# peterropac/Aegolius

Hardware: AMD Instinct MI355X
Metric: Mpoints/sec SDF eval, 1024^3 grid, 10-prim smooth-union tree (higher is better)
Workload: dtype f32

## Files before the change

### aegolius_amd/_engine.py

```python
import atexit
import contextlib
import ctypes
import importlib.util
import os
import sys
import threading

import numpy as np

_HERE = os.path.dirname(os.path.abspath(__file__))
LIB_PATH = os.path.join(_HERE, "libsdfk.so")

MODE_AUTO, MODE_INTERPRET, MODE_SPECIALIZED, MODE_NOCULL = 0, 1, 2, 3
(FLAVOUR_PLAIN_ARRAY, FLAVOUR_PLAIN_GRID, FLAVOUR_TILE_ARRAY, FLAVOUR_TILE_GRID, FLAVOUR_TILE_MASK, FLAVOUR_ROWS_ARRAY,
 FLAVOUR_ROWS_GRID, FLAVOUR_ROWS_MASK, FLAVOUR_ROWS2D_ARRAY, FLAVOUR_ROWS2D_GRID, FLAVOUR_RAYS, FLAVOUR_OCCUPANCY) = range(12)
FLAVOUR_FLAGS = 0x100
FLAVOUR_XY = 0x200

_c = ctypes
_vp, _i64, _int, _sz = _c.c_void_p, _c.c_int64, _c.c_int, _c.c_size_t
_fp = _c.POINTER(_c.c_float)

SIGNATURES = {
    "sdfk_abi_version": (_int, []),
    "sdfk_device_count": (_int, []),
    "sdfk_last_error": (_c.c_char_p, []),
    "sdfk_program_create": (_vp, [_vp, _sz, _vp, _sz, _vp, _sz, _int]),
    "sdfk_program_destroy": (None, [_vp]),
    "sdfk_program_set_params": (_int, [_vp, _vp, _sz]),
    "sdfk_program_set_cull": (_int, [_vp, _vp, _sz, _vp]),
    "sdfk_program_source": (_c.c_char_p, [_vp]),
    "sdfk_program_compile_check": (_int, [_vp, _c.POINTER(_sz)]),
    "sdfk_program_chain_members": (_int, [_vp]),
    "sdfk_program_compile_flavour": (_int, [_vp, _int, _c.POINTER(_sz), _c.POINTER(_c.c_double)]),
    "sdfk_debug_compile_external": (_int, [_vp, _int, _c.POINTER(_sz)]),
    "sdfk_debug_jit_stats": (None, [_c.POINTER(_i64), _c.POINTER(_c.c_double)]),
    "sdfk_jit_drain": (None, []),
    "sdfk_jit_cancel": (None, []),
    "sdfk_debug_set_rtc_defs": (None, [_c.c_char_p]),
    "sdfk_eval_device": (_int, [_vp, _vp, _i64, _i64, _vp, _vp, _int]),
    "sdfk_eval_device_rows": (_int, [_vp, _vp, _i64, _i64, _i64, _vp, _vp, _int]),
    "sdfk_eval_device_rows2d": (_int, [_vp, _vp, _i64, _i64, _i64, _vp, _vp, _int]),
    "sdfk_eval_device_rows2d_xy": (_int, [_vp, _vp, _i64, _i64, _i64, _vp, _vp, _int]),
    "sdfk_debug_cells_stats": (None, [_int, _c.POINTER(_c.c_longlong)]),
    "sdfk_debug_rays_stats": (None, [_int, _c.POINTER(_c.c_longlong)]),
    "sdfk_eval_device_rows3d": (_int, [_vp, _vp, _i64, _i64, _i64, _i64, _i64, _vp, _vp, _int]),
    "sdfk_debug_row_masks": (_int, [_vp, _vp, _i64, _i64, _i64, _vp, _c.POINTER(_i64), _c.POINTER(_int), _vp]),
    "sdfk_eval_grid_sharded": (_int, [_vp, _vp, _i64, _vp, _i64, _vp, _i64, _int, _vp, _vp, _int]),
    "sdfk_eval_grid_sharded_device": (_int, [_vp, _vp, _i64, _vp, _i64, _vp, _i64, _int, _vp, _int, _vp, _int]),
    "sdfk_eval_device_aux": (_int, [_vp, _vp, _i64, _i64, _vp, _int, _i64, _vp, _vp, _int]),
    "sdfk_eval_grid_aux": (_int, [_vp, _vp, _i64, _vp, _i64, _vp, _i64, _i64, _i64, _vp, _int, _i64, _vp, _vp, _int]),
    "sdfk_field_min": (_int, [_vp, _i64, _c.POINTER(_c.c_float), _vp]),
    "sdfk_grid_box_average": (_int, [_vp, _i64, _i64, _i64, _int, _int, _int, _int, _vp, _vp]),
    "sdfk_grid_edge_detect": (_int, [_vp, _i64, _i64, _i64, _vp, _vp]),
    "sdfk_debug_box_variant": (_int, [_i64, _i64, _i64, _int, _int, _int, _c.POINTER(_int)]),
    "sdfk_grid_signed": (_int, [_vp, _i64, _i64, _i64, _c.c_float, _int, _vp, _vp]),
    "sdfk_grid_boundary_mask": (_int, [_vp, _i64, _c.c_float, _vp, _vp]),
    "sdfk_grid_signed_slab": (_int, [_vp, _i64, _i64, _vp, _i64, _i64, _i64, _int, _vp, _vp]),
    "sdfk_eval_host": (_int, [_vp, _vp, _int, _i64, _i64, _vp, _int, _int]),
    "sdfk_eval_host_resident": (_int, [_vp, _vp, _int, _i64, _i64, _vp, _int, _int]),
    "sdfk_field_select_scratch": (_sz, [_i64]),
    "sdfk_field_select": (_int, [_vp, _i64, _c.c_float, _vp, _i64, _c.POINTER(_i64), _vp, _vp]),
    "sdfk_field_select_finish": (_int, [_i64, _i64, _vp, _i64, _vp, _vp]),
    "sdfk_field_gradient": (_int, [_vp, _i64, _i64, _i64, _int, _int, _vp, _i64, _vp]),
    "sdfk_field_crossings_2d": (_int, [_vp, _vp, _i64, _i64, _i64, _c.c_double, _c.c_double, _c.c_double, _vp, _vp]),
    "sdfk_lcwg_eval": (_int, [_int, _vp, _vp, _i64, _i64, _i64, _c.c_double, _c.c_double, _int, _c.c_double, _vp, _vp, _i64,
                              _vp]),
    "sdfk_lcwg_old_eval": (_int, [_int, _vp, _i64, _vp, _i64, _c.c_double, _c.c_double, _vp, _i64, _vp]),
    "sdfk_eval_select_scratch": (_sz, [_i64, _i64]),
    "sdfk_eval_device_select": (_int, [_vp, _vp, _i64, _i64, _i64, _int, _c.c_float, _vp, _i64, _c.POINTER(_i64), _vp, _vp, _int]),
    "sdfk_eval_grid_select": (_int, [_vp, _vp, _i64, _vp, _i64, _vp, _i64, _i64, _i64, _c.c_float, _vp, _i64, _c.POINTER(_i64),
                                     _vp, _vp, _int]),
    "sdfk_eval_select_finish": (_int, [_vp, _i64, _i64, _int, _i64, _vp, _i64, _vp, _vp]),
    "sdfk_vec_eval_device": (_int, [_vp, _int, _vp, _i64, _i64, _vp, _int, _i64, _int, _vp, _i64, _vp]),
    "sdfk_vec_set_interpret": (None, [_int]),
    "sdfk_vec_source": (_c.c_char_p, [_vp, _int, _int, _int]),
    "sdfk_vec_compile_check": (_int, [_vp, _int, _int, _int, _c.POINTER(_sz)]),
    "sdfk_vec_eval_host": (_int, [_vp, _int, _vp, _int, _i64, _vp, _i64, _vp, _i64, _vp, _i64, _vp, _int, _int, _vp, _int]),
    "sdfk_eval_grid": (_int, [_vp, _vp, _i64, _vp, _i64, _vp, _i64, _i64, _i64, _vp, _vp, _int]),
    "sdfk_eval_grid_host": (_int, [_vp, _vp, _i64, _vp, _i64, _vp, _i64, _i64, _i64, _vp, _int, _int]),
    "sdfk_set_default_mode": (None, [_int]),
    "sdfk_debug_brick_masks": (_int, [_vp, _vp, _i64, _i64, _vp, _vp]),
    "sdfk_linspace_f32": (_int, [_c.c_double, _c.c_double, _i64, _vp]),
    "sdfk_point_tree_build": (_i64, [_vp, _i64, _int, _vp, _i64, _vp, _vp, _vp]),
    "sdfk_grid_fill": (_int, [_vp, _i64, _vp, _i64, _vp, _i64, _vp, _i64, _i64, _i64, _vp]),
    "sdfk_set_device": (_int, [_int]),
    "sdfk_malloc": (_vp, [_sz]),
    "sdfk_free": (_int, [_vp]),
    "sdfk_memcpy_h2d": (_int, [_vp, _vp, _sz]),
    "sdfk_memcpy_d2h": (_int, [_vp, _vp, _sz]),
    "sdfk_memcpy_d2d": (_int, [_vp, _vp, _sz]),
    "sdfk_sync": (_int, [_vp]),
    "sdfk_event_create": (_vp, []),
    "sdfk_event_destroy": (_int, [_vp]),
    "sdfk_event_record": (_int, [_vp, _vp]),
    "sdfk_event_elapsed_ms": (_int, [_vp, _vp, _fp]),
    "sdfk_stream_probe": (_int, [_vp, _i64, _i64, _vp, _vp]),
    "sdfk_dual_has_rule": (_int, [_int]),
    "sdfk_program_jvp_check": (_int, [_vp, _c.POINTER(_int)]),
    "sdfk_eval_jvp_device": (_int, [_vp, _vp, _i64, _i64, _vp, _int, _int, _vp, _vp, _i64, _vp]),
    "sdfk_value_jvp_device": (_int, [_int, _vp, _vp, _vp, _i64, _vp, _vp, _vp]),
    "sdfk_program_vjp_check": (_int, [_vp, _c.POINTER(_int), _c.POINTER(_i64)]),
    "sdfk_vjp_limits": (_int, [_c.POINTER(_int), _c.POINTER(_int)]),
    "sdfk_eval_vjp_device": (_int, [_vp, _vp, _i64, _i64, _vp, _int, _int, _vp, _vp, _vp, _vp]),
    "sdfk_points_bin": (_int, [_vp, _i64, _i64, _vp, _i64, _i64, _i64, _vp, _vp]),
    "sdfk_points_extent": (_int, [_vp, _i64, _i64, _i64, _vp, _vp]),
    "sdfk_points_fill": (_int, [_vp, _i64, _i64, _i64, _int, _i64, _i64, _i64, _vp]),
    "sdfk_points_widen": (_int, [_vp, _i64, _int, _vp, _vp]),
    "sdfk_field_isosurface_scratch": (_sz, [_i64, _i64, _i64]),
    "sdfk_field_isosurface": (_int, [_vp, _vp, _i64, _vp, _i64, _vp, _i64, _c.c_float, _c.POINTER(_i64), _c.POINTER(_i64), _vp,
                                     _vp]),
    "sdfk_field_isosurface_finish": (_int, [_vp, _i64, _i64, _i64, _c.c_float, _i64, _i64, _vp, _i64, _vp, _i64, _int, _vp,
                                            _vp]),
    "sdfk_field_contour2d_scratch": (_sz, [_i64, _i64]),
    "sdfk_field_contour2d": (_int, [_vp, _vp, _i64, _vp, _i64, _c.c_float, _c.POINTER(_i64), _c.POINTER(_i64), _vp, _vp]),
    "sdfk_field_contour2d_finish": (_int, [_vp, _i64, _i64, _c.c_float, _i64, _i64, _vp, _i64, _vp, _i64, _int, _vp, _vp]),
    "sdfk_eval_grid_isosurface_scratch": (_sz, [_i64, _i64, _i64]),
    "sdfk_eval_grid_isosurface": (_int, [_vp, _vp, _i64, _vp, _i64, _vp, _i64, _c.c_float, _c.POINTER(_i64), _c.POINTER(_i64),
                                         _vp, _vp, _int]),
    "sdfk_eval_grid_isosurface_finish": (_int, [_vp, _vp, _i64, _vp, _i64, _vp, _i64, _c.c_float, _i64, _i64, _vp, _i64, _vp,
                                                _i64, _int, _vp, _vp, _int]),
    "sdfk_eval_grid_contour2d_scratch": (_sz, [_i64, _i64]),
# ... 660 lines not shown
```

### aegolius_amd/csrc/sdfk.hip

```cpp
#include <hip/hip_runtime.h>
#include <hip/hiprtc.h>

#include <chrono>
#include <algorithm>
#include <atomic>
#include <cmath>
#include <condition_variable>
#include <cstdio>
#include <cstdlib>
#include <cstring>
#include <deque>
#include <functional>
#include <map>
#include <memory>
#include <mutex>
#include <thread>
#include <string>
#include <vector>
#include <dirent.h>
#include <dlfcn.h>
#include <fcntl.h>
#include <signal.h>
#include <spawn.h>
#include <sys/wait.h>
// ... 985 lines not shown
        std::unique_lock<std::mutex> lk(mu);
        cv.wait(lk, [this] { return jobs.empty() && busy == 0; });
    }
    void drop_queued() {
        std::lock_guard<std::mutex> lk(mu);
        jobs.clear();
        cv.notify_all();
    }
    ~BuildWorker() {
        {
            std::lock_guard<std::mutex> lk(mu);
            stop = true;
            cv.notify_all();
        }
        for (std::thread& t : threads)
            if (t.joinable()) t.join();
    }
};
static BuildWorker g_builds;
extern "C" void sdfk_jit_drain(void) { g_builds.drain(); }
extern "C" void sdfk_jit_cancel(void) {
    g_cancel_builds.store(true);
    g_builds.drop_queued();
    g_builds.drain();
}
static std::atomic<long long> g_compile_count{0};
static std::atomic<long long> g_compile_micros{0};
extern "C" void sdfk_debug_jit_stats(int64_t* builds, double* seconds) {
    if (builds) *builds = g_compile_count.load();
    if (seconds) *seconds = (double)g_compile_micros.load() * 1e-6;
}

static std::shared_ptr<CodeObject> code_entry(const std::string& key) {
    std::lock_guard<std::mutex> lk(g_code_mu);
    std::shared_ptr<CodeObject>& e = g_code[key];
    if (!e) e = std::make_shared<CodeObject>();
    return e;
}
static void code_build(const std::shared_ptr<CodeObject>& e, const std::string& src, int rwb, bool external = false) {
    const auto t0 = std::chrono::steady_clock::now();
    std::vector<char> co;
    std::string log;
    bool from_disk = false;
    std::string disk_path;
    const int rc = rtc_compile(src, &co, &log, rwb, &from_disk, &disk_path, external);
    const double dt = std::chrono::duration<double>(std::chrono::steady_clock::now() - t0).count();
    if (!from_disk) {
        g_compile_count++;
        g_compile_micros += (long long)(dt * 1e6);
    }
    std::lock_guard<std::mutex> lk(e->mu);
    e->build_seconds = dt;
    if (rc == 0) {
        e->co.swap(co);
        e->disk_path = disk_path;
        e->state = 2;
    } else {
        e->error = log;
        e->state = 3;
        e->failed_at = std::chrono::steady_clock::now();
    }
    e->cv.notify_all();
}
template <typename MakeSource>
static std::shared_ptr<CodeObject> code_get(const std::string& key, MakeSource make_source, int rwb, bool wait) {
    std::shared_ptr<CodeObject> e = code_entry(key);
    std::unique_lock<std::mutex> lk(e->mu);
    if (e->state == 3 && std::chrono::steady_clock::now() - e->failed_at > std::chrono::seconds(30)) e->state = 0;
    if (e->state == 0) {
        e->state = 1;
        lk.unlock();
        const std::string src = make_source();
        if (wait || !rtc_helper_available()) {
            code_build(e, src, rwb);
        } else {
            g_builds.post([e, src, rwb] { code_build(e, src, rwb, true); });
        }
        return e;
    }
    if (wait) e->cv.wait(lk, [&] { return e->state != 1; });
    return e;
}
static std::string flavour_key(const sdfk_program* p, int flavour, int rwb, int with_flags = 0) {
    return p->key + "|f" + std::to_string(flavour) + ((with_flags & 1) ? "s" : "") + ((with_flags & 2) ? "x" : "") + "|" + rtc_option_key(rwb);
}
static std::string flavour_source(const sdfk_program* p, int flavour, int with_flags = 0) {
    return std::string((with_flags & 1) ? "#define SDFK_FLAGS 1\n" : "") + ((with_flags & 2) ? "#define SDFK_XY 1\n" : "") +
           sdfk_generate_source(g_ops, SDFK_OP_COUNT, p->code.data(), p->code.size() / 2, p->result_reg, p->sites, flavour,
                                &p->sites_all);
}

extern "C" int sdfk_program_chain_members(const sdfk_program* p) {
    return p && p->chain_mode ? p->chain_members : 0;
}
extern "C" int sdfk_program_compile_check(sdfk_program* p, size_t* code_size) {
    if (!p) return fail(-1, "null program");
    size_t total = 0;
    const int rwb = rows_geo(p);
    for (int f = 0; f < SDFK_FL_COUNT; ++f) {
        if (f == SDFK_FL_RAYS) continue;
        if (f == SDFK_FL_OCCUPANCY) continue;
        if (p->sites.empty() && f != SDFK_FL_PLAIN_ARRAY && f != SDFK_FL_PLAIN_GRID) continue;
        if (p->chain_mode && (f == SDFK_FL_TILE_ARRAY || f == SDFK_FL_TILE_GRID || f == SDFK_FL_TILE_MASK || f == SDFK_FL_ROWS_MASK)) continue;
        std::shared_ptr<CodeObject> e = code_get(flavour_key(p, f, rwb), [&] { return flavour_source(p, f); }, rwb, true);
        if (e->state != 2) return fail(-3, e->error);
        total += e->co.size();
    }
    if (code_size) *code_size = total;
    return 0;
}
extern "C" int sdfk_program_compile_flavour(sdfk_program* p, int flavour, size_t* code_size, double* seconds) {
    if (!p) return fail(-1, "null program");
    int with_flags = 0;
    if (flavour >= 0 && (flavour & SDFK_FLAVOUR_FLAGS)) with_flags |= 1;
    if (flavour >= 0 && (flavour & SDFK_FLAVOUR_XY)) with_flags |= 2;
    if (flavour >= 0) flavour &= ~(SDFK_FLAVOUR_FLAGS | SDFK_FLAVOUR_XY);
    if (flavour < 0 || flavour >= SDFK_FL_COUNT) return fail(-1, "sdfk_program_compile_flavour: unknown flavour");
    if (p->sites.empty() && flavour != SDFK_FL_PLAIN_ARRAY && flavour != SDFK_FL_PLAIN_GRID && flavour != SDFK_FL_RAYS &&
        flavour != SDFK_FL_OCCUPANCY)
        return fail(-2, "sdfk_program_compile_flavour: the program has no cull sites");
    if (with_flags && flavour == SDFK_FL_RAYS)
        return fail(-2, "sdfk_program_compile_flavour: the ray flavour has no flag-writing or two-row build");
    if (with_flags && flavour == SDFK_FL_OCCUPANCY)
        return fail(-2, "sdfk_program_compile_flavour: the occupancy flavour has no flag-writing or two-row build");
    if ((with_flags & 2) && flavour != SDFK_FL_PLAIN_ARRAY && flavour != SDFK_FL_ROWS2D_ARRAY)
        return fail(-2, "sdfk_program_compile_flavour: two-row coordinates exist for the plain and the flat row-block array kernels");
    if ((with_flags & 1) && (flavour == SDFK_FL_TILE_ARRAY || flavour == SDFK_FL_TILE_GRID || flavour == SDFK_FL_TILE_MASK ||
                       flavour == SDFK_FL_ROWS_MASK))
        return fail(-2, "sdfk_program_compile_flavour: this flavour has no flag-writing build");
    const int rwb = rows_geo(p);
    const auto t0 = std::chrono::steady_clock::now();
    std::shared_ptr<CodeObject> e =
        code_get(flavour_key(p, flavour, rwb, with_flags), [&] { return flavour_source(p, flavour, with_flags); }, rwb, true);
    if (e->state != 2) return fail(-3, e->error);
    if (code_size) *code_size = e->co.size();
    if (seconds) *seconds = std::chrono::duration<double>(std::chrono::steady_clock::now() - t0).count();
    return 0;
}

extern "C" int sdfk_debug_compile_external(sdfk_program* p, int flavour, size_t* code_size) {
    if (!p) return fail(-1, "null program");
    if (flavour < 0 || flavour >= SDFK_FL_COUNT) return fail(-1, "sdfk_debug_compile_external: unknown flavour");
    if (p->sites.empty() && flavour != SDFK_FL_PLAIN_ARRAY && flavour != SDFK_FL_PLAIN_GRID && flavour != SDFK_FL_RAYS &&
        flavour != SDFK_FL_OCCUPANCY)
        return fail(-2, "sdfk_debug_compile_external: the program has no cull sites");
    if (!rtc_helper_available()) return fail(-9, "sdfk_rtc_helper is not next to libsdfk.so (or hiprtc cannot be located)");
    std::vector<char> co;
    std::string log;
    if (rtc_compile_external(flavour_source(p, flavour), &co, &log, rows_geo(p)) != 0) return fail(-3, log);
    if (code_size) *code_size = co.size();
    return 0;
}

static std::shared_ptr<SpecModule> get_module(sdfk_program* p, int device, int flavour, bool wait, std::string* err,
                                              int with_flags = 0) {
    const int rwb = rows_geo(p);
    const std::string key = flavour_key(p, flavour, rwb, with_flags);
    std::shared_ptr<SpecModule> m;
    {
        std::lock_guard<std::mutex> lk(g_code_mu);
        std::shared_ptr<SpecModule>& slot = g_mods[std::make_pair(device, key)];
        if (!slot) slot = std::make_shared<SpecModule>();
        m = slot;
    }
    std::lock_guard<std::mutex> lk(m->mu);
    if (m->loaded) return m;
    for (int attempt = 0;; ++attempt) {
        std::shared_ptr<CodeObject> e;
        {
            std::lock_guard<std::mutex> ce(g_code_mu);
// ... 177 lines not shown
                 o_head = (o_cspan + 8 * nc + 63) & ~(size_t)63, o_pool = o_head + 2 * 64 * shards, total = o_pool + 4 * cap + 64;
    CellScratch* cs;
    {
        std::lock_guard<std::mutex> lk(p->mu);
        cs = &d->cells[stream];
    }
    if (cs->bytes < total) {
        if (cs->buf) {
            HIPCHK(hipStreamSynchronize(stream));
            (void)hipFree(cs->buf);
            cs->buf = nullptr;
            cs->bytes = 0;
        }
        if (hipMalloc(&cs->buf, total + total / 4) != hipSuccess) { (void)hipGetLastError(); return 0; }
        cs->bytes = total + total / 4;
    }
    char* b = cs->buf;
    HIPCHK(hipMemsetAsync(b + o_head, 0, 2 * 64 * shards, stream));
    CellPassArg cp{};
    cp.cand = b + o_pool;
    if (coarse) {
        cp.lv = crs; cp.parent = CellLevelH{}; cp.sph = b + o_csph; cp.span = b + o_cspan; cp.psph = nullptr; cp.pspan = nullptr;
        cp.ncells = (unsigned)nc; cp.inflate = 1.3f;
        cp.head = reinterpret_cast<unsigned*>(b + o_head);
        cp.base = 0u; cp.shard_cap = (unsigned)cshard;
        std::vector<void*> args = {(void*)&prm, (void*)&tab};
        for (int i = 0; i < n_src; ++i) args.push_back(src[i]);
        RowGeom g2 = rg;
        args.push_back(&g2);
        args.push_back(&cp);
        HIPCHK(hipModuleLaunchKernel(cells_fn, (unsigned)((nc + 3) / 4), 1, 1, 256, 1, 1, 0, stream, args.data(), nullptr));
    }
    cp.lv = fine; cp.parent = coarse ? crs : CellLevelH{}; cp.sph = b + o_fsph; cp.span = b + o_fspan;
    cp.psph = coarse ? b + o_csph : nullptr; cp.pspan = coarse ? b + o_cspan : nullptr;
    cp.ncells = (unsigned)nf; cp.inflate = 1.0f;
    cp.head = reinterpret_cast<unsigned*>(b + o_head + 64 * shards);
    cp.base = (unsigned)(shards * cshard); cp.shard_cap = (unsigned)fshard;
    {
        std::vector<void*> args = {(void*)&prm, (void*)&tab};
        for (int i = 0; i < n_src; ++i) args.push_back(src[i]);
        RowGeom g2 = rg;
        args.push_back(&g2);
        args.push_back(&cp);
        HIPCHK(hipModuleLaunchKernel(cells_fn, (unsigned)((nf + 3) / 4), 1, 1, 256, 1, 1, 0, stream, args.data(), nullptr));
    }
    static const bool trace = [] { const char* e = getenv("SDFK_CELLS_TRACE"); return e && e[0] == '1'; }();
    if (trace || g_cells_stats_on.load()) {
        HIPCHK(hipStreamSynchronize(stream));
        std::vector<uint2> sp(nf);
        unsigned head = 0;
        HIPCHK(hipMemcpy(sp.data(), b + o_fspan, 8 * nf, hipMemcpyDeviceToHost));
        {
            std::vector<unsigned> heads(2 * 16 * shards);
            HIPCHK(hipMemcpy(heads.data(), b + o_head, 2 * 64 * shards, hipMemcpyDeviceToHost));
            for (size_t i = 0; i < heads.size(); i += 16) head += heads[i];
        }
        unsigned long long sum = 0, all = 0, empty = 0, mx = 0;
        for (const uint2& x : sp) {
            if (x.y == 0xffffffffu) ++all;
            else { sum += x.y; mx = std::max<unsigned long long>(mx, x.y); if (x.y == 0) ++empty; }
        }
        {
            std::lock_guard<std::mutex> lk(g_cells_stats_mu);
            g_cells_stats[0] = (long long)nf; g_cells_stats[1] = (long long)nc; g_cells_stats[2] = (long long)head;
            g_cells_stats[3] = (long long)cap; g_cells_stats[4] = (long long)sum; g_cells_stats[5] = (long long)mx;
            g_cells_stats[6] = (long long)all; g_cells_stats[7] = (long long)empty;
        }
        if (trace) fprintf(stderr, "[sdfk cells] %d members: fine %ux%ux%u = %llu cells (2^%u planes x 2^%u blocks x 2^%u windows), coarse %llu; pool %u of %llu entries; "
                "fine lists: mean %.1f max %llu, %llu without a list, %llu empty\n", p->chain_members, fine.ncx, fine.ncy, fine.ncz, nf, fine.lx, fine.ly, fine.lz, nc,
                head, cap, (double)sum / (double)std::max<unsigned long long>(1, nf - all - empty), mx, all, empty);
    }
    out->lv = fine;
    out->sph = b + o_fsph;
    out->span = b + o_fspan;
    out->cand = b + o_pool;
    out->enabled = 1u;
    out->ncells = (unsigned)nf;
    return 0;
}

static int run(sdfk_program* p, const SrcArray* arr, const SrcGrid* grid, long long n, float* d_out, void* stream_,
               int mode, bool vec_ok, long long row_len = 0, const float* aux = nullptr, long long aux_stride = 0,
               bool flat = false, long long plane_rows = 0, long long plane_phase = 0, unsigned* d_flags = nullptr,
               unsigned thr_key = 0, bool xy = false) {
    if (!p) return fail(-1, "null program");
    if (n < 0) return fail(-1, "negative point count");
    if (p->n_aux > 0 && (!aux || aux_stride < n))
        return fail(-1, "this program reads auxiliary fields (staged evaluation): use sdfk_eval_device_aux / sdfk_eval_grid_aux");
    if (n == 0) return 0;
    if (mode == SDFK_MODE_AUTO) mode = g_default_mode;
    if (d_flags && (mode == SDFK_MODE_AUTO || mode == SDFK_MODE_INTERPRET)) mode = SDFK_MODE_SPECIALIZED;
    if (xy) {
        if (!arr || p->n_aux > 0) return fail(-1, "two-row coordinates: array source, no auxiliary fields");
        if (mode == SDFK_MODE_AUTO || mode == SDFK_MODE_INTERPRET) mode = SDFK_MODE_SPECIALIZED;
    }
    hipStream_t stream = (hipStream_t)stream_;
    int device = 0;
    HIPCHK(hipGetDevice(&device));
    DevState* d = nullptr;
    int rc = ensure_resident(p, device, stream, &d);
    if (rc) return rc;

    long long n4 = vec_ok ? (n / 4) * 4 : 0;
    long long tail = n - n4;

    static const long long spec_limit = [] {
        const char* e = getenv("SDFK_SPECIALIZE_LIMIT");
        const long long v = e ? atoll(e) : 1200;
        return v > 0 ? v : 1200;
    }();
    static const long long rows_limit = [] {
        const char* e = getenv("SDFK_ROWS_LIMIT");
        const long long v = e ? atoll(e) : 1200;
        return v > 0 ? v : 1200;
    }();
    if (mode == SDFK_MODE_AUTO && (long long)(p->code.size() / 2) > spec_limit && p->interp_ok && !p->chain_mode && !d_flags)
        mode = SDFK_MODE_INTERPRET;

    RowGeom rg;
    int flavour = arr ? SDFK_FL_PLAIN_ARRAY : SDFK_FL_PLAIN_GRID;
    const long long grow = grid ? (grid->n2 > 1 ? (long long)grid->n2 : (long long)grid->n1) : 0;
    if (!p->sites.empty() && mode != SDFK_MODE_NOCULL && mode != SDFK_MODE_INTERPRET) {
        if (arr && rows_geometry(n, row_len, &rg, (flat || d_flags) ? 0 : plane_rows, plane_phase, p->chain_mode))
            flavour = (flat || xy) ? SDFK_FL_ROWS2D_ARRAY : SDFK_FL_ROWS_ARRAY;
        else if (arr && vec_ok && !p->chain_mode && !d_flags && !xy) flavour = SDFK_FL_TILE_ARRAY;
        else if (grid && grid->start % grow == 0 &&
                 rows_geometry(n, grow, &rg, (grid->n2 > 1 && !d_flags) ? (long long)grid->n1 : 0,
                               grid->n2 > 1 ? (grid->start / grow) % (long long)grid->n1 : 0, p->chain_mode))
            flavour = grid->n2 > 1 ? SDFK_FL_ROWS_GRID : SDFK_FL_ROWS2D_GRID;
        else if (grid && vec_ok && !p->chain_mode && !d_flags) flavour = SDFK_FL_TILE_GRID;
        if (!p->chain_mode && (long long)(p->code.size() / 2) > rows_limit &&
            (flavour == SDFK_FL_ROWS_ARRAY || flavour == SDFK_FL_ROWS2D_ARRAY || flavour == SDFK_FL_ROWS_GRID || flavour == SDFK_FL_ROWS2D_GRID)) {
            const bool is_arr = arr != nullptr;
            if (vec_ok && !d_flags && !xy) flavour = is_arr ? SDFK_FL_TILE_ARRAY : SDFK_FL_TILE_GRID;
            else if (!d_flags) flavour = is_arr ? SDFK_FL_PLAIN_ARRAY : SDFK_FL_PLAIN_GRID;
        }
    }
    std::shared_ptr<SpecModule> sk;
    if (mode != SDFK_MODE_INTERPRET) {
        static const bool async_jit = [] { const char* e = getenv("SDFK_ASYNC_JIT"); return !(e && e[0] == '0'); }();
        const bool wait = mode != SDFK_MODE_AUTO || !p->interp_ok || !async_jit;
        std::string err;
        sk = get_module(p, device, flavour, wait, &err, (d_flags ? 1 : 0) | (xy ? 2 : 0));
        if (sk && sk->failed) {
            if (mode == SDFK_MODE_SPECIALIZED || !p->interp_ok)
                return fail(-3, "specialised kernel unavailable: " + err);
            static bool warned = false;
            if (!warned) {
                fprintf(stderr, "[sdfk] hiprtc specialisation failed, using the interpreter kernel: %s\n", err.c_str());
                warned = true;
            }
            sk.reset();
        }
    }
    if (!sk && !p->interp_ok)
        return fail(-4, "program needs more registers than the interpreter kernel has (use the specialised mode)");

    const float* prm = d->d_params;
    const float* tab = d->d_tables;
    if (sk) {
        if (flavour == SDFK_FL_ROWS_ARRAY || flavour == SDFK_FL_ROWS_GRID || flavour == SDFK_FL_ROWS2D_ARRAY ||
            flavour == SDFK_FL_ROWS2D_GRID) {
            const unsigned per_tile = (unsigned)(rows_waves(p) * rows_wbricks(p));
            const unsigned tiles = ((rg.nbricks + per_tile - 1) / per_tile + 127u) & ~127u;
            const unsigned rthreads = 64u * (unsigned)rows_waves(p);
            CellsArg cells{};
            const bool with_cells = p->chain_mode && sk->fn[1] != nullptr;
            if (arr) {
                const float* co = arr->co;
                long long stride = arr->stride;
                if (with_cells) {
                    void* src[] = {&co, &stride};
                    rc = prepare_cells(p, d, sk->fn[1], rg, src, 2, prm, tab, stream, &cells);
                    if (rc) return rc;
                }
                void* args[] = {&prm, &tab, &co, &stride, &rg, &d_out, &d_flags, &thr_key, &cells};
                HIPCHK(hipModuleLaunchKernel(sk->fn[0], tiles, 1, 1, rthreads, 1, 1, 0, stream, args, nullptr));
            } else {
                SrcGrid g = *grid;
                rg.row0 = grid->start / grow;
                rg.yrows = grid->n2 > 1 ? 0 : 1;
                if (with_cells) {
                    void* src[] = {&g};
                    rc = prepare_cells(p, d, sk->fn[1], rg, src, 1, prm, tab, stream, &cells);
                    if (rc) return rc;
                }
                void* args[] = {&prm, &tab, &g, &rg, &d_out, &d_flags, &thr_key, &cells};
                HIPCHK(hipModuleLaunchKernel(sk->fn[0], tiles, 1, 1, rthreads, 1, 1, 0, stream, args, nullptr));
            }
            return 0;
        }
        if (flavour == SDFK_FL_TILE_ARRAY || flavour == SDFK_FL_TILE_GRID) {
            const unsigned tiles = (unsigned)((n + tile_points() - 1) / tile_points());
            if (arr) {
                const float* co = arr->co;
                long long stride = arr->stride;
                void* args[] = {&prm, &tab, &co, &stride, &n, &d_out};
                HIPCHK(hipModuleLaunchKernel(sk->fn[0], tiles, 1, 1, tile_threads(), 1, 1, 0, stream, args, nullptr));
            } else {
                SrcGrid g = *grid;
                void* args[] = {&prm, &tab, &g, &n, &d_out};
                HIPCHK(hipModuleLaunchKernel(sk->fn[0], tiles, 1, 1, tile_threads(), 1, 1, 0, stream, args, nullptr));
            }
            return 0;
        }
        if (arr) {
            const float* co = arr->co;
            long long stride = arr->stride;
            if (n4) {
                long long off = 0;
                void* args[] = {&prm, &tab, &co, &stride, &off, &n4, &d_out, &aux, &aux_stride, &d_flags, &thr_key};
                HIPCHK(hipModuleLaunchKernel(sk->fn[0], blocks_for(n4, 4), 1, 1, SDFK_BLOCK, 1, 1, 0, stream, args,
                                             nullptr));
            }
            if (tail) {
                long long off = n4;
                void* args[] = {&prm, &tab, &co, &stride, &off, &tail, &d_out, &aux, &aux_stride, &d_flags, &thr_key};
                HIPCHK(hipModuleLaunchKernel(sk->fn[1], blocks_for(tail, 1), 1, 1, SDFK_BLOCK, 1, 1, 0, stream, args,
                                             nullptr));
            }
        } else {
            SrcGrid g = *grid;
            if (n4) {
                long long off = 0;
                void* args[] = {&prm, &tab, &g, &off, &n4, &d_out, &aux, &aux_stride, &d_flags, &thr_key};
                HIPCHK(hipModuleLaunchKernel(sk->fn[0], blocks_for(n4, 4), 1, 1, SDFK_BLOCK, 1, 1, 0, stream, args,
                                             nullptr));
            }
            if (tail) {
                long long off = n4;
                void* args[] = {&prm, &tab, &g, &off, &tail, &d_out, &aux, &aux_stride, &d_flags, &thr_key};
                HIPCHK(hipModuleLaunchKernel(sk->fn[1], blocks_for(tail, 1), 1, 1, SDFK_BLOCK, 1, 1, 0, stream, args,
                                             nullptr));
            }
        }
        return 0;
    }
    if (d_flags) return fail(-3, "fused selection needs the specialised kernels");
    const int n_instr = (int)(p->code.size() / 2);
    const long long zero = 0;
    auto launch = [&](auto src, int vec, long long off, long long cnt) {
        using SRC = decltype(src);
        const dim3 grid(blocks_for(cnt, vec)), block(SDFK_BLOCK);
#define SDFK_INTERP_GO(VEC, NC, NV) hipLaunchKernelGGL((sdfk_interp_kernel<VEC, NC, NV, SRC>), grid, block, 0, stream, d->d_code, \
                                                        n_instr, prm, tab, src, off, cnt, d_out, p->result_reg, aux, aux_stride)
        if (vec == 4) {
            if (p->interp_small) SDFK_INTERP_GO(4, SDFK_NC_SMALL, SDFK_NV_SMALL);
            else SDFK_INTERP_GO(4, SDFK_NC, SDFK_NV);
        } else {
            if (p->interp_small) SDFK_INTERP_GO(1, SDFK_NC_SMALL, SDFK_NV_SMALL);
            else SDFK_INTERP_GO(1, SDFK_NC, SDFK_NV);
        }
#undef SDFK_INTERP_GO
    };
    if (arr) {
        if (n4) launch(*arr, 4, zero, n4);
        if (tail) launch(*arr, 1, n4, tail);
    } else {
        if (n4) launch(*grid, 4, zero, n4);
        if (tail) launch(*grid, 1, n4, tail);
    }
    HIPCHK(hipGetLastError());
    return 0;
}

static bool aligned16(const void* p) { return (reinterpret_cast<uintptr_t>(p) & 15u) == 0; }

extern "C" int sdfk_eval_device(sdfk_program* p, const float* d_co, int64_t n, int64_t row_stride, float* d_out,
                                void* stream, int mode) {
    if (!d_co || !d_out) return fail(-1, "sdfk_eval_device: null device pointer");
// ... 54 lines not shown
    if (!p || !d_co || !d_out) return fail(-1, "sdfk_eval_device_aux: null pointer");
    if (row_stride < n) return fail(-1, "sdfk_eval_device_aux: row stride smaller than the point count");
    if (n_aux < p->n_aux) return fail(-1, "sdfk_eval_device_aux: the program reads more auxiliary fields than were passed");
    SrcArray a = {d_co, (long long)row_stride};
    bool vec_ok = aligned16(d_co) && aligned16(d_out) && (row_stride % 4 == 0);
    return run(p, &a, nullptr, n, d_out, stream, mode, vec_ok, 0, d_aux, aux_stride);
}

extern "C" int sdfk_debug_row_masks(sdfk_program* p, const float* d_co, int64_t n, int64_t row_stride, int64_t row_len,
                                    uint64_t* d_masks, int64_t* n_bricks, int* brick_rows, void* stream_) {
    if (!p || !d_co) return fail(-1, "sdfk_debug_row_masks: null argument");
    if (p->sites.empty()) return fail(-2, "sdfk_debug_row_masks: program has no cull sites");
    if (p->chain_mode) return fail(-2, "sdfk_debug_row_masks: a chain-mode program keeps lists of surviving children, not mask words");
    RowGeom rg;
    if (row_stride < n || !rows_geometry(n, row_len, &rg))
        return fail(-1, "sdfk_debug_row_masks: the row-block kernel does not take this shape");
    if (n_bricks) *n_bricks = rg.nbricks;
    if (brick_rows) *brick_rows = 16;
    if (!d_masks) return 0;
    hipStream_t stream = (hipStream_t)stream_;
    int device = 0;
    HIPCHK(hipGetDevice(&device));
    DevState* d = nullptr;
    int rc = ensure_resident(p, device, stream, &d);
    if (rc) return rc;
    std::string err;
    std::shared_ptr<SpecModule> sk = get_module(p, device, SDFK_FL_ROWS_MASK, true, &err);
    if (!sk || sk->failed) return fail(-3, "specialised kernel unavailable: " + err);
    const float* prm = d->d_params;
    const float* tab = d->d_tables;
    long long stride = row_stride;
    void* args[] = {&prm, &tab, &d_co, &stride, &rg, &d_masks};
    const unsigned per_tile = (unsigned)(rows_waves(p) * rows_wbricks(p));
    HIPCHK(hipModuleLaunchKernel(sk->fn[0], (rg.nbricks + per_tile - 1) / per_tile, 1, 1, 64 * rows_waves(p), 1, 1, 0, stream,
                                 args, nullptr));
    return 0;
}

extern "C" int sdfk_debug_brick_masks(sdfk_program* p, const float* d_co, int64_t n, int64_t row_stride,
                                      uint64_t* d_masks, void* stream_) {
    if (!p || !d_co || !d_masks) return fail(-1, "sdfk_debug_brick_masks: null argument");
    if (!(aligned16(d_co) && row_stride % 4 == 0 && row_stride >= n && n > 0))
        return fail(-1, "sdfk_debug_brick_masks: needs 16-byte aligned rows");
    if (p->sites.empty()) return fail(-2, "sdfk_debug_brick_masks: program has no cull sites");
    if (p->chain_mode) return fail(-2, "sdfk_debug_brick_masks: chain-mode programs have no line-brick flavour");
    hipStream_t stream = (hipStream_t)stream_;
    int device = 0;
    HIPCHK(hipGetDevice(&device));
    DevState* d = nullptr;
    int rc = ensure_resident(p, device, stream, &d);
    if (rc) return rc;
    std::string err;
    std::shared_ptr<SpecModule> sk = get_module(p, device, SDFK_FL_TILE_MASK, true, &err);
    if (!sk || sk->failed) return fail(-3, "specialised kernel unavailable: " + err);
    const float* prm = d->d_params;
    const float* tab = d->d_tables;
    long long stride = row_stride, nn = n;
    void* args[] = {&prm, &tab, &d_co, &stride, &nn, &d_masks};
    HIPCHK(hipModuleLaunchKernel(sk->fn[0], (unsigned)((n + tile_points() - 1) / tile_points()), 1, 1, tile_threads(),
                                 1, 1, 0, stream, args, nullptr));
    return 0;
}

extern "C" int sdfk_linspace_f32(double lo, double hi, int64_t n, float* out) {
    if (n < 0 || (n > 0 && !out)) return fail(-1, "sdfk_linspace_f32: bad arguments");
    if (n == 0) return 0;
    if (n == 1) {
        out[0] = (float)lo;
        return 0;
    }
    const double div = (double)(n - 1);
    const double delta = hi - lo;
    const double step = delta / div;
    for (int64_t i = 0; i < n; ++i) {
        volatile double t = (step != 0.0) ? (double)i * step : ((double)i / div) * delta;
        out[i] = (float)(t + lo);
    }
    out[n - 1] = (float)hi;
    return 0;
}

struct AxisTables {
    float* d = nullptr;
    ~AxisTables() {
        if (d) (void)hipFree(d);
    }
};

static int upload_axes(const float* ax0, int64_t n0, const float* ax1, int64_t n1, const float* ax2, int64_t n2,
                       hipStream_t stream, AxisTables* t, SrcGrid* g, int64_t start) {
    if (!ax0 || !ax1 || !ax2 || n0 < 1 || n1 < 1 || n2 < 1) return fail(-1, "grid axes missing or empty");
    if (n1 > 0x7fffffff || n2 > 0x7fffffff) return fail(-1, "grid axis too long");
    HIPCHK(hipMalloc(&t->d, (size_t)(n0 + n1 + n2) * sizeof(float)));
    HIPCHK(hipMemcpyAsync(t->d, ax0, (size_t)n0 * sizeof(float), hipMemcpyHostToDevice, stream));
    HIPCHK(hipMemcpyAsync(t->d + n0, ax1, (size_t)n1 * sizeof(float), hipMemcpyHostToDevice, stream));
    HIPCHK(hipMemcpyAsync(t->d + n0 + n1, ax2, (size_t)n2 * sizeof(float), hipMemcpyHostToDevice, stream));
    g->ax0 = t->d;
    g->ax1 = t->d + n0;
    g->ax2 = t->d + n0 + n1;
    g->n1 = (unsigned)n1;
    g->n2 = (unsigned)n2;
    g->start = start;
    return 0;
}

extern "C" int sdfk_eval_grid(sdfk_program* p, const float* ax0, int64_t n0, const float* ax1, int64_t n1,
                              const float* ax2, int64_t n2, int64_t start, int64_t count, float* d_out, void* stream,
                              int mode) {
    if (!d_out) return fail(-1, "sdfk_eval_grid: null output");
    if (start < 0 || count < 0 || start + count > n0 * n1 * n2) return fail(-1, "sdfk_eval_grid: range outside the grid");
    AxisTables t;
    SrcGrid g;
    int rc = upload_axes(ax0, n0, ax1, n1, ax2, n2, (hipStream_t)stream, &t, &g, start);
    if (rc) return rc;
    rc = run(p, nullptr, &g, count, d_out, stream, mode, aligned16(d_out));
    if (rc) return rc;
    HIPCHK(hipStreamSynchronize((hipStream_t)stream));
    return 0;
}

extern "C" int sdfk_eval_grid_aux(sdfk_program* p, const float* ax0, int64_t n0, const float* ax1, int64_t n1,
                                  const float* ax2, int64_t n2, int64_t start, int64_t count, const float* d_aux, int n_aux,
                                  int64_t aux_stride, float* d_out, void* stream, int mode) {
    if (!p || !d_out) return fail(-1, "sdfk_eval_grid_aux: null pointer");
    if (start < 0 || count < 0 || start + count > n0 * n1 * n2) return fail(-1, "sdfk_eval_grid_aux: range outside the grid");
    if (n_aux < p->n_aux) return fail(-1, "sdfk_eval_grid_aux: the program reads more auxiliary fields than were passed");
    AxisTables t;
    SrcGrid g;
    int rc = upload_axes(ax0, n0, ax1, n1, ax2, n2, (hipStream_t)stream, &t, &g, start);
    if (rc) return rc;
    rc = run(p, nullptr, &g, count, d_out, stream, mode, aligned16(d_out), 0, d_aux, aux_stride);
    if (rc) return rc;
    HIPCHK(hipStreamSynchronize((hipStream_t)stream));
    return 0;
}

extern "C" int sdfk_eval_grid_host(sdfk_program* p, const float* ax0, int64_t n0, const float* ax1, int64_t n1,
                                   const float* ax2, int64_t n2, int64_t start, int64_t count, float* out, int device,
                                   int mode) {
    if (!p) return fail(-1, "null program");
    if (count < 0 || (count > 0 && !out)) return fail(-1, "sdfk_eval_grid_host: bad arguments");
    if (start < 0 || start + count > n0 * n1 * n2) return fail(-1, "sdfk_eval_grid_host: range outside the grid");
    if (count == 0) return 0;
    HIPCHK(hipSetDevice(device));
    int64_t chunk = std::min<int64_t>(count, (int64_t)1 << 27);
    const int64_t grow = n2 > 1 ? n2 : n1;
    if (start % grow == 0 && chunk > grow) chunk = chunk / grow * grow;
    float* d_out = nullptr;
    HIPCHK(hipMalloc(&d_out, (size_t)chunk * sizeof(float)));
    AxisTables t;
    SrcGrid g;
    int rc = upload_axes(ax0, n0, ax1, n1, ax2, n2, nullptr, &t, &g, start);
    for (int64_t s = 0; s < count && rc == 0; s += chunk) {
        const int64_t m = std::min(chunk, count - s);
        g.start = start + s;
        rc = run(p, nullptr, &g, m, d_out, nullptr, mode, true);
        if (rc == 0 && hipMemcpy(out + s, d_out, (size_t)m * sizeof(float), hipMemcpyDeviceToHost) != hipSuccess)
            rc = fail(-6, "sdfk_eval_grid_host: device-to-host copy failed");
    }
    (void)hipFree(d_out);
    return rc;
}

extern "C" int sdfk_eval_grid_sharded(sdfk_program* p, const float* ax0, int64_t n0, const float* ax1, int64_t n1,
                                      const float* ax2, int64_t n2, int n_shards, const int* devices, float* out,
                                      int mode) {
    if (!p || !out) return fail(-1, "sdfk_eval_grid_sharded: null argument");
    if (n_shards < 1 || n_shards > 64) return fail(-1, "sdfk_eval_grid_sharded: 1..64 shards");
    if (!ax0 || !ax1 || !ax2 || n0 < 1 || n1 < 1 || n2 < 1) return fail(-1, "grid axes missing or empty");
    int n_dev = 0;
    if (hipGetDeviceCount(&n_dev) != hipSuccess || n_dev < 1) return fail(-8, "sdfk_eval_grid_sharded: no HIP device");
    const int64_t total = n0 * n1 * n2, unit = n2 > 1 ? n2 : n1;
    const int64_t per = (total / unit / n_shards) * unit;
    std::vector<int> rc((size_t)n_shards, 0);
    std::vector<std::string> msg((size_t)n_shards);
    std::vector<std::thread> workers;
    for (int d = 0; d < n_shards; ++d) {
        const int dev = devices ? devices[d] : d % n_dev;
        if (dev < 0 || dev >= n_dev) return fail(-1, "sdfk_eval_grid_sharded: device index out of range");
    }
    for (int d = 0; d < n_shards; ++d) {
        const int dev = devices ? devices[d] : d % n_dev;
        const int64_t start = d * per, count = d < n_shards - 1 ? per : total - start;
        workers.emplace_back([=, &rc, &msg] {
            rc[(size_t)d] = count > 0 ? sdfk_eval_grid_host(p, ax0, n0, ax1, n1, ax2, n2, start, count, out + start, dev, mode) : 0;
            if (rc[(size_t)d]) msg[(size_t)d] = sdfk_last_error();
        });
    }
    for (std::thread& t : workers) t.join();
    for (int d = 0; d < n_shards; ++d)
        if (rc[(size_t)d]) return fail(rc[(size_t)d], "shard " + std::to_string(d) + ": " + msg[(size_t)d]);
    return 0;
}

extern "C" int sdfk_eval_grid_sharded_device(sdfk_program* p, const float* ax0, int64_t n0, const float* ax1, int64_t n1,
                                             const float* ax2, int64_t n2, int n_shards, const int* devices,
                                             int gather_device, float* d_full, int mode) {
    if (!p || !d_full) return fail(-1, "sdfk_eval_grid_sharded_device: null argument");
    if (n_shards < 1 || n_shards > 64) return fail(-1, "sdfk_eval_grid_sharded_device: 1..64 shards");
    if (!ax0 || !ax1 || !ax2 || n0 < 1 || n1 < 1 || n2 < 1) return fail(-1, "grid axes missing or empty");
    int n_dev = 0;
    if (hipGetDeviceCount(&n_dev) != hipSuccess || n_dev < 1) return fail(-8, "sdfk_eval_grid_sharded_device: no HIP device");
    if (gather_device < 0 || gather_device >= n_dev) return fail(-1, "sdfk_eval_grid_sharded_device: gather device out of range");
    for (int d = 0; d < n_shards; ++d) {
        const int dev = devices ? devices[d] : d % n_dev;
        if (dev < 0 || dev >= n_dev) return fail(-1, "sdfk_eval_grid_sharded_device: device index out of range");
    }
    const int64_t total = n0 * n1 * n2, unit = n2 > 1 ? n2 : n1;
    const int64_t per = (total / unit / n_shards) * unit;
    std::vector<int> rc((size_t)n_shards, 0);
    std::vector<std::string> msg((size_t)n_shards);
    std::vector<std::thread> workers;
    for (int d = 0; d < n_shards; ++d) {
        const int dev = devices ? devices[d] : d % n_dev;
        const int64_t start = d * per, count = d < n_shards - 1 ? per : total - start;
        workers.emplace_back([=, &rc, &msg] {
            auto shard = [&]() -> int {
                if (count <= 0) return 0;
                HIPCHK(hipSetDevice(dev));
                hipStream_t stream = nullptr;
                HIPCHK(hipStreamCreateWithFlags(&stream, hipStreamNonBlocking));
                static const bool force_copy = [] { const char* e = getenv("SDFK_FORCE_PEER_COPY"); return e && e[0] == '1'; }();
                const bool in_place = dev == gather_device && !force_copy;
                float* d_slab = in_place ? d_full + start : nullptr;
                int r = 0;
                if (!d_slab && hipMalloc(&d_slab, (size_t)count * sizeof(float)) != hipSuccess) r = fail(-5, "out of device memory for the slab");
                if (r == 0) r = sdfk_eval_grid(p, ax0, n0, ax1, n1, ax2, n2, start, count, d_slab, stream, mode);
                if (r == 0 && !in_place) {
                    if (hipMemcpyPeerAsync(d_full + start, gather_device, d_slab, dev, (size_t)count * sizeof(float), stream) != hipSuccess ||
                        hipStreamSynchronize(stream) != hipSuccess)
                        r = fail(-6, "peer copy of the slab failed");
                }
                if (!in_place && d_slab) (void)hipFree(d_slab);
                (void)hipStreamDestroy(stream);
                return r;
            };
            rc[(size_t)d] = shard();
            if (rc[(size_t)d]) msg[(size_t)d] = sdfk_last_error();
        });
// ... 300 lines not shown
```

### aegolius_amd/csrc/sdfk_access.h

```cpp
#ifndef SDFK_ACCESS_H
#define SDFK_ACCESS_H

#define SDFK_BLOCK 256

struct SrcArray {
    const float* __restrict__ co;
    long long stride;
};
struct SrcGrid {
    const float* __restrict__ ax0;
    const float* __restrict__ ax1;
    const float* __restrict__ ax2;
    unsigned n1, n2;
    long long start;
};

typedef float sdfk_f4 __attribute__((ext_vector_type(4)));
static __device__ __forceinline__ float4 sdfk_stream_load4(const float* p) {
    const sdfk_f4 v = __builtin_nontemporal_load(reinterpret_cast<const sdfk_f4*>(p));
    return make_float4(v.x, v.y, v.z, v.w);
}
static __device__ __forceinline__ void sdfk_stream_store4(float* p, float a, float b, float c, float d) {
    const sdfk_f4 v = {a, b, c, d};
    __builtin_nontemporal_store(v, reinterpret_cast<sdfk_f4*>(p));
}

template <int VEC>
static __device__ __forceinline__ void sdfk_load(const SrcArray& s, long long block_base, unsigned lane_off,
                                                 V3 (&p)[VEC]) {
    const long long i = block_base + lane_off;
    if constexpr (VEC == 4) {
        const float4 x = sdfk_stream_load4(s.co + i);
        const float4 y = sdfk_stream_load4(s.co + s.stride + i);
#ifdef SDFK_XY
        const float4 z = make_float4(0.0f, 0.0f, 0.0f, 0.0f);
#else
        const float4 z = sdfk_stream_load4(s.co + 2 * s.stride + i);
#endif
        p[0] = {x.x, y.x, z.x};
        p[1] = {x.y, y.y, z.y};
        p[2] = {x.z, y.z, z.z};
        p[3] = {x.w, y.w, z.w};
    } else {
#pragma unroll
#ifdef SDFK_XY
        for (int v = 0; v < VEC; ++v) p[v] = {s.co[i + v], s.co[s.stride + i + v], 0.0f};
#else
        for (int v = 0; v < VEC; ++v) p[v] = {s.co[i + v], s.co[s.stride + i + v], s.co[2 * s.stride + i + v]};
#endif
    }
}

template <int VEC>
static __device__ __forceinline__ void sdfk_load(const SrcGrid& s, long long block_base, unsigned lane_off,
                                                 V3 (&p)[VEC]) {
    const unsigned long long base = (unsigned long long)(s.start + block_base);
    const unsigned long long row = base / s.n2;
    const unsigned iz0 = (unsigned)(base - row * s.n2);
    const unsigned long long ix0 = row / s.n1;
    const unsigned iy0 = (unsigned)(row - ix0 * s.n1);
#pragma unroll
    for (int v = 0; v < VEC; ++v) {
        const unsigned t = iz0 + lane_off + v;
        const unsigned cz = t / s.n2;
        const unsigned iz = t - cz * s.n2;
        const unsigned ty = iy0 + cz;
        const unsigned cy = ty / s.n1;
        const unsigned iy = ty - cy * s.n1;
        p[v] = {s.ax0[ix0 + cy], s.ax1[iy], s.ax2[iz]};
    }
}

static __host__ __device__ __forceinline__ unsigned sdfk_sel_key(float v) {
    unsigned u = __builtin_bit_cast(unsigned, v);
    if ((u & 0x7fffffffu) > 0x7f800000u) return 0xffffffffu;
    if (u == 0x80000000u) u = 0u;
    return (u & 0x80000000u) ? ~u : (u | 0x80000000u);
}
template <int VEC>
static __device__ __forceinline__ void sdfk_store_flags(unsigned* __restrict__ flags, long long i, unsigned nib, bool active) {
    if constexpr (VEC == 4) {
        const unsigned lane = __builtin_amdgcn_workitem_id_x() & 63u;
        unsigned w = nib << (4u * (lane & 7u));
        w |= __shfl_xor(w, 1);
        w |= __shfl_xor(w, 2);
        w |= __shfl_xor(w, 4);
        if ((lane & 7u) == 0u && active) flags[i >> 5] = w;
    } else {
        if (active && nib) atomicOr(&flags[i >> 5], nib << (unsigned)(i & 31));
    }
}

template <int VEC>
static __device__ __forceinline__ void sdfk_store(float* __restrict__ out, long long i, const float (&v)[VEC]) {
    if constexpr (VEC == 4) {
        sdfk_stream_store4(out + i, v[0], v[1], v[2], v[3]);
    } else {
#pragma unroll
// ... 6 lines not shown
```

### aegolius_amd/csrc/sdfk_codegen.cpp

```cpp
#include "sdfk_codegen.h"

#include <algorithm>
#include <cstdio>
#include <cstring>
#include <map>
#include <set>

#include "sdfk_embedded.inc"

std::string sdfk_vector_prelude() { return std::string(kEmbeddedDevice) + "\n" + kEmbeddedVecdev + "\n"; }

static const char kWrappers[] = R"SDFKW(
template <int VEC, typename SRC>
static __device__ __forceinline__ void sdfk_body(const float* __restrict__ PRM, const float* __restrict__ TAB,
                                                 const SRC& src, long long off, long long n,
                                                 float* __restrict__ out, const float* __restrict__ aux,
                                                 long long aux_stride, unsigned* __restrict__ flags, unsigned thr) {
    const long long block_base = (long long)sdfk_bx() * (SDFK_BLOCK * VEC);
    const unsigned lane_off = sdfk_tx() * VEC;
#ifdef SDFK_FLAGS                                              // the flag-writing build of this flavour (its own code object:
    {                                                          // carried as a run-time branch it cost the field kernels registers)
        const bool active = block_base + lane_off < n;
        unsigned nib = 0u;
        if (active) {
// ... 565 lines not shown
}
)SDFKT";
static const char kTileArray[] = R"SDFKT(
extern "C" __global__ __launch_bounds__(SDFK_TTHREADS) void sdfk_spec_t(
    const float* __restrict__ PRM, const float* __restrict__ TAB, const float* __restrict__ co, long long stride,
    long long n, float* __restrict__ out) {
    const SrcArray s = {co, stride};
    sdfk_tile_kernel(PRM, TAB, s, n, out);
}
)SDFKT";
static const char kTileGrid[] = R"SDFKT(
// the same on a regular grid expanded from three per-axis tables: no coordinate array at all (4 B/point)
extern "C" __global__ __launch_bounds__(SDFK_TTHREADS) void sdfk_spec_tg(
    const float* __restrict__ PRM, const float* __restrict__ TAB, SrcGrid g, long long n, float* __restrict__ out) {
    sdfk_tile_kernel(PRM, TAB, g, n, out);
}
)SDFKT";
static const char kTileMask[] = R"SDFKT(
// debugging / test aid: the skip masks of every brick (2 bits per site: bit 2k = skip first operand,
// bit 2k+1 = skip second operand; bit 63 = x/y-constant run, bit 62 = two such runs)
extern "C" __global__ __launch_bounds__(SDFK_TTHREADS) void sdfk_spec_tmask(
    const float* __restrict__ PRM, const float* __restrict__ TAB, const float* __restrict__ co, long long stride,
    long long n, unsigned long long* __restrict__ masks) {
    __shared__ __attribute__((aligned(16))) sdfk_tilemeta meta;
    const SrcArray s = {co, stride};
    sdfk_tile_prepare(PRM, TAB, s, n, &meta);
    for (int b = sdfk_tx(); b < SDFK_NBRICK; b += SDFK_TTHREADS)
        masks[(long long)sdfk_bx() * SDFK_NBRICK + b] = sdfk_brick_mask(&meta, b);
}
)SDFKT";


static const char kSimtGeometry[] = R"SDFKR(
#ifndef SDFK_RWBRICKS
#define SDFK_RWBRICKS 2
#endif
#ifndef SDFK_RWAVES
#define SDFK_RWAVES 4
#endif
#ifndef SDFK_NSUB                        // sub-bricks (probe centres) per brick: 16 = 4 rows x 8 points, 8 = 8 rows x 8, 4 = 16 rows x 8
// becomes the cost: 4 centres up to 96 leaves (round 4, smooth unions of n primitives at 513^3, 1 -> 4 centres: n = 40
#define SDFK_NSUB ((SDFK_NLEAF <= 32 && 8 * SDFK_RWBRICKS <= 64) ? 8 : ((SDFK_NLEAF <= 96 && 4 * SDFK_RWBRICKS <= 64) ? 4 : 1))
#endif
#define SDFK_NCEN (SDFK_RWAVES * SDFK_RWBRICKS * SDFK_NSUB)
static_assert(SDFK_NSUB == 1 || SDFK_NSUB == 4 || SDFK_NSUB == 8 || SDFK_NSUB == 16, "1, 4, 8 or 16 probe centres per brick");
static_assert(SDFK_NCEN <= 64 * SDFK_RWAVES, "one fold lane per probe centre");
)SDFKR";

static const char kRowsKernel[] = R"SDFKR(
#ifndef SDFK_RWBRICKS
#define SDFK_RWBRICKS 2
#endif
#ifndef SDFK_RWAVES
#define SDFK_RWAVES 4                           // waves per workgroup (host launch code must agree: sdfk.hip)
#endif
#define SDFK_RZ 32
#define SDFK_RLPR (SDFK_RZ / (2 * SDFK_NP))     // lanes per row in phase C
#define SDFK_RROWS (64 / SDFK_RLPR)             // rows per brick
#define SDFK_RBRICK (SDFK_RZ * SDFK_RROWS)
#define SDFK_RLOADS (SDFK_RROWS / 8)            // load instructions per array and brick
#define SDFK_RNBRICK (SDFK_RWAVES * SDFK_RWBRICKS)
#ifndef SDFK_CHUNK
#define SDFK_CHUNK 16                            // chain mode: children whose parameters are staged in LDS at a time
#endif
#ifndef SDFK_STAGE_MIN
#define SDFK_STAGE_MIN 2                         // ... when more than this many survive on the brick
#endif
#ifndef SDFK_CHAIN_STAGED                        // Round 3 staged the survivors' parameters in LDS for chains of more than 64
#define SDFK_CHAIN_STAGED 0                      // children (three dependent loads per child: kind, base, parameters). With the
#endif                                           // survivors kept as RECORDS (round 4) one load is left between the list and the
                                                 // 4096: 2.21 -> 2.11 (SDFK_STAGE_MIN=64 against 2); -DSDFK_CHAIN_STAGED=1 brings it back
static_assert(SDFK_NP == 2 || SDFK_NP == 4, "2 or 4 packed pairs per lane");
static_assert(SDFK_RNBRICK <= 64 * SDFK_RWAVES, "one probe lane per brick");

typedef float sdfk_f4u __attribute__((ext_vector_type(4), aligned(4)));

#ifdef SDFK_CELLS
#ifndef SDFK_ALIST_CAP
#define SDFK_ALIST_CAP (SDFK_NLEAF < 192 ? SDFK_NLEAF : 192)     // survivors a brick's list holds in LDS
#endif
#define SDFK_ALL_ALIVE 0xffffffffu
#define SDFK_LIST_ALIVE 0xfffffffeu
#endif
struct sdfk_rowmeta {
    float z[SDFK_RNBRICK][SDFK_RBRICK];         // [row of the brick][point of the window]
    float2 xy[SDFK_RNBRICK][SDFK_RROWS];
    float4 bound[SDFK_RNBRICK];
    unsigned long long mask[SDFK_NMASK][SDFK_RNBRICK];   // two bits per site: SDFK_NMASK x 32 sites (2 words up to 64 sites)
    unsigned uniform[SDFK_RNBRICK];
#if defined(SDFK_SIMT) && !defined(SDFK_CELLS)
    float4 cen[SDFK_NCEN];                      // probe centres (x, y, z, radius): SDFK_NSUB per brick
    float leafval[SDFK_NLEAF * SDFK_NCEN];      // [leaf][centre]: every leaf of the tree at every centre
#endif
#ifdef SDFK_CHAIN
#ifdef SDFK_CELLS
    unsigned alist[SDFK_RNBRICK][SDFK_ALIST_CAP];                      // RECORDS of the children that run, in order
    uint2 aspan[SDFK_RNBRICK];                                         // more survivors than that: the cell's whole list runs (nalive = LIST)
    unsigned inside[SDFK_RNBRICK];                                     // every point of the brick lies in its cell's sphere
#else
    unsigned short alist[SDFK_RNBRICK][SDFK_NLEAF];                    // the children that run, in order
#endif
    unsigned nalive[SDFK_RNBRICK];
#if SDFK_CHAIN_STAGED
    float cprm[SDFK_RNBRICK][SDFK_CHUNK][SDFK_NPLMAX];                  // parameters of the chunk of children being evaluated
    unsigned cgrp[SDFK_RNBRICK][SDFK_CHUNK];                            // ... and their kinds
#endif
#endif
#ifdef SDFK_LDSPAD
    float pad[SDFK_LDSPAD / 4];                 // experiment: a larger LDS footprint per workgroup
#endif
};
struct sdfk_rowgeom {
    unsigned L, nchunk, nbricks;                // row length, windows per row, bricks in total
    long long R;                                // rows
    long long row0;                             // grid flavour: global row index of the first row of the slab
    int yrows;                                  // grid flavour, 2-D grid (n2 == 1): rows run along the second axis
    unsigned prow, seg0, nb0, bpp;              // planes of prow rows after a first partial plane of seg0 rows (nb0 blocks);
                                                // bpp blocks per plane: a block never holds rows of two planes
    unsigned inv_nchunk, inv_bpp;               // floor(2^32 / nchunk), floor(2^32 / bpp): divisions as one v_mul_hi
};
#ifdef SDFK_CELLS
// Candidate lists (chain mode). The bricks are grouped into CELLS in index space — 2^lx plane slots x 2^ly row blocks x
// 2^lz windows — and a pre-pass (sdfk_spec_cells) leaves per cell a bounding sphere, derived from the coordinates of the
// cell's eight corner points, and the LIST of members that can be the minimum somewhere in that sphere (the global-minimum
// rule of sdfk_chain_fold at the cell's radius; cells of a coarser level first, so that a fine cell only looks at its
// parent's list). A brick then probes the members on its cell's list instead of all of them — after checking, point by
// point, that it really lies inside the sphere: the corner points bound the cell only if the array is the lattice its
// layout hints say it is, and a brick that fails the check (or whose cell ran out of list space) probes every member,
// as before. Whatever the input, a member that is dropped cannot be the minimum at any point of the brick.
struct sdfk_celllevel {
    unsigned lx, ly, lz;                        // log2 of the cell size in plane slots, row blocks, windows
    unsigned ncx, ncy, ncz;                     // cells along each of them
    unsigned xoff;                              // slot number of the first whole plane (2^lx when a partial plane leads, else 0)
    unsigned pad;
};
struct sdfk_cells {
    sdfk_celllevel lv;                          // the level the bricks look at (the finest)
    const float4* __restrict__ sph;             // per cell: centre, radius (< 0: no such cell)
    const uint2* __restrict__ span;             // per cell: first entry, entries (SDFK_ALL_ALIVE: no list — probe every member)
    const unsigned* __restrict__ cand;          // the lists: one RECORD per member (sdfk_member_record: kind and parameter block)
    unsigned enabled, ncells;
};
#endif
// a / d for wave-uniform a, with inv = floor(2^32 / d) from the host: the estimate is never too large and at most a few
// units too small (a * (2^32 - inv * d) < 2^32 * d for every brick count the host accepts), the loop repairs it.
// (A plain 32-bit division is ~35 vector instructions; this kernel has two per brick.)
static __device__ __forceinline__ unsigned sdfk_udiv(unsigned a, unsigned d, unsigned inv) {
    unsigned q = __umulhi(a, inv);
    while (a - q * d >= d) ++q;
    return __builtin_amdgcn_readfirstlane(q);
}
// rows [r0, rend) of row block rb (wave-uniform): 16 consecutive rows of ONE plane, fewer at the end of a plane
// (slot, blk: plane slot — 0 = the leading partial plane, whole planes from 0 as well; the caller adds its offset — and the
//  block's index within it)
static __device__ __forceinline__ void sdfk_block_rows(const sdfk_rowgeom& g, unsigned rb, long long& r0, long long& rend,
                                                       unsigned* slot = nullptr, unsigned* blk = nullptr) {
    // ONE plane (no plane hint, flat grids, plane blocks not asked for): blocks of 16 consecutive rows, nothing to divide
    if (g.nb0 == 0u && (long long)g.prow >= g.R) {
        r0 = (long long)rb * SDFK_RROWS;
        rend = g.R;
        if (slot) { *slot = 0u; *blk = rb; }
        return;
    }
    if (rb < g.nb0) {
        r0 = (long long)rb * SDFK_RROWS;
        rend = g.seg0;
        if (slot) { *slot = 0xffffffffu; *blk = rb; }
    } else {
// ... 18 lines not shown
    if (interior) {
        const sdfk_f4u v = __builtin_nontemporal_load(reinterpret_cast<const sdfk_f4u*>(rowp + z));
        return make_float4(v.x, v.y, v.z, v.w);
    }
    // edge window, branch-free on purpose: per-lane branches around the loads (whole quad / one value / mixed)
    return make_float4(rowp[min(max(z, 0), last)], rowp[min(max(z + 1, 0), last)], rowp[min(max(z + 2, 0), last)],
                       rowp[min(max(z + 3, 0), last)]);
}
// the 4 points [z, z+4) of row `row` (row = r0 + dr, r0 wave-uniform) as three quads
static __device__ __forceinline__ void sdfk_rows_fetch(const SrcArray& s, const sdfk_rowgeom& g, long long r0, int dr, int z,
                                                       bool interior, float4& X, float4& Y, float4& Z) {
    const float* p = s.co + (r0 + dr) * (long long)g.L;
    const int last = (int)g.L - 1;
    X = sdfk_win_quad(p, z, last, interior);
    Y = sdfk_win_quad(p + s.stride, z, last, interior);
#ifdef SDFK_XY                                                    // two-row coordinates (z = 0 by contract): 12 B/point
    Z = make_float4(0.0f, 0.0f, 0.0f, 0.0f);
#else
    Z = sdfk_win_quad(p + 2 * s.stride, z, last, interior);
#endif
}
// regular grid: row -> (ix, iy) with one wave-uniform division per brick; z from the third axis table
static __device__ __forceinline__ void sdfk_rows_fetch(const SrcGrid& s, const sdfk_rowgeom& g, long long r0, int dr, int z,
                                                       bool interior, float4& X, float4& Y, float4& Z) {
    const unsigned long long g0 = (unsigned long long)(g.row0 + r0);
    if (g.yrows) {                                                 // (x, y, z) = (ax0[row], ax1[point], ax2[0])
        const float x = s.ax0[g0 + (unsigned)dr], zc = s.ax2[0];
        X = make_float4(x, x, x, x);
        Y = sdfk_win_quad(s.ax1, z, (int)g.L - 1, interior);
        Z = make_float4(zc, zc, zc, zc);
        return;
    }
    unsigned long long ix = g0 / s.n1;
    unsigned iy = (unsigned)(g0 - ix * s.n1) + (unsigned)dr;
    while (iy >= s.n1) { iy -= s.n1; ++ix; }
    const float x = s.ax0[ix], y = s.ax1[iy];
    X = make_float4(x, x, x, x);
    Y = make_float4(y, y, y, y);
    Z = sdfk_win_quad(s.ax2, z, (int)g.L - 1, interior);
}
static __device__ __forceinline__ float sdfk_prev_lane(float v) {   // value of lane-1 within a row of 16 lanes
    return __builtin_bit_cast(float, __builtin_amdgcn_update_dpp(__builtin_bit_cast(int, v), __builtin_bit_cast(int, v), 0x111, 0xf, 0xf, false));
}
// point index (in its row) of the first point of window k of local row `row`, plus e0
static __device__ __forceinline__ int sdfk_win_z(long long row, unsigned L, unsigned k, int e0, long long* flat) {
    const long long rl = row * (long long)L;
    const long long f = (((rl >> 5) + k) << 5) + e0;
    *flat = f;
    return (int)(f - rl);
}

// phase A, part 1: issue the loads of one brick (wave-uniform r0, k); 8 rows x 32 points per instruction
struct sdfk_rowregs {
    float4 X[SDFK_RLOADS], Y[SDFK_RLOADS], Z[SDFK_RLOADS];
};
template <typename SRC>
static __device__ __forceinline__ void sdfk_rows_load(const SRC& s, const sdfk_rowgeom& g, long long r0, long long rend,
                                                      unsigned k, int lane, sdfk_rowregs& r) {
    // SDFK_FLAT (flat grids: rows run along y, z = 0 everywhere): the roles of y and z are swapped from here to the
    // end of phase A — r.Y holds z (the coordinate a row shares, which must be exactly 0) and r.Z holds y (the one
    // that varies along the row) — so that "uniform", the staging and the bounding sphere work unchanged
    const bool interior = sdfk_interior(g.L, k);
#pragma unroll
    for (int t = 0; t < SDFK_RLOADS; ++t) {
        int dr = 8 * t + (lane >> 3);
        if (r0 + dr >= rend) dr = (int)(rend - 1 - r0);
        long long flat;
        const int z = sdfk_win_z(r0 + dr, g.L, k, 4 * (lane & 7), &flat);
        #ifdef SDFK_FLAT
        sdfk_rows_fetch(s, g, r0, dr, z, interior, r.X[t], r.Z[t], r.Y[t]);
#else
        sdfk_rows_fetch(s, g, r0, dr, z, interior, r.X[t], r.Y[t], r.Z[t]);
#endif
    }
}
// phase A, part 2: z and the row heads to LDS, "every row has one x and one y", bounding sphere
// (SDFK_CELLS: S = sphere of the brick's cell, with y and z swapped for SDFK_FLAT like the registers; the brick also learns
//  whether every one of its points lies inside it)
#ifdef SDFK_CELLS
#define SDFK_CELL_ARG , float4 S
#else
#define SDFK_CELL_ARG
#endif
static __device__ __forceinline__ void sdfk_rows_bounds(const sdfk_rowregs& r, int lane, sdfk_rowmeta* meta, int b SDFK_CELL_ARG) {
#ifdef SDFK_ABLATE_BOUNDS
    *reinterpret_cast<float4*>(&meta->z[b][(lane >> 3) * SDFK_RZ + 4 * (lane & 7)]) = r.Z[0];
    if (SDFK_RLOADS > 1) *reinterpret_cast<float4*>(&meta->z[b][(8 + (lane >> 3)) * SDFK_RZ + 4 * (lane & 7)]) = r.Z[SDFK_RLOADS - 1];
    if ((lane & 7) == 0) { meta->xy[b][lane >> 3] = make_float2(r.X[0].x, r.Y[0].x); meta->xy[b][SDFK_RROWS - 8 + (lane >> 3)] = make_float2(r.X[SDFK_RLOADS - 1].x, r.Y[SDFK_RLOADS - 1].x); }
    if (lane == 0) { meta->bound[b] = make_float4(0.f, 0.f, 0.f, 1.f); meta->uniform[b] = 1u; }
#ifdef SDFK_CELLS
    if (lane == 0) meta->inside[b] = S.w > 0.0f ? 1u : 0u;
#endif
    return;
#endif
    bool uni = true;
#pragma unroll
    for (int t = 0; t < SDFK_RLOADS; ++t) {
        *reinterpret_cast<float4*>(&meta->z[b][(8 * t + (lane >> 3)) * SDFK_RZ + 4 * (lane & 7)]) = r.Z[t];
        const float px = sdfk_prev_lane(r.X[t].x), py = sdfk_prev_lane(r.Y[t].x);
        const bool head = (lane & 7) == 0;
        uni = uni && r.X[t].x == r.X[t].y && r.X[t].x == r.X[t].z && r.X[t].x == r.X[t].w && r.Y[t].x == r.Y[t].y &&
              r.Y[t].x == r.Y[t].z && r.Y[t].x == r.Y[t].w && (head || (px == r.X[t].x && py == r.Y[t].x));
#ifdef SDFK_FLAT
        uni = uni && r.Y[t].x == 0.0f;                             // (M2 * 0 drops out of every root transform exactly)
#endif
        if (head) meta->xy[b][8 * t + (lane >> 3)] = make_float2(r.X[t].x, r.Y[t].x);
    }
    const bool uniform = __ballot(uni) == ~0ull;
#if defined(SDFK_SIMT) && SDFK_NSUB > 1
    // bricks of whole row segments are bounded per SUB-brick by the probe lanes (sdfk_sub_centre, from the staged
    // coordinates): the sphere around the whole brick is only needed for the others
    if (uniform) {
        if (lane == 0) {
            meta->uniform[b] = 1u;
#pragma unroll
            for (int w = 0; w < SDFK_NMASK; ++w) meta->mask[w][b] = ~0ull;
        }
        return;
    }
#endif
    const float cx = 0.5f * (sdfk_lane(r.X[0].x, 0) + sdfk_lane(r.X[SDFK_RLOADS - 1].w, 63));
    const float cy = 0.5f * (sdfk_lane(r.Y[0].x, 0) + sdfk_lane(r.Y[SDFK_RLOADS - 1].w, 63));
    const float cz = 0.5f * (sdfk_lane(r.Z[0].x, 0) + sdfk_lane(r.Z[SDFK_RLOADS - 1].w, 63));
    float d2 = 0.0f;
#ifdef SDFK_CELLS
    float d2s = 0.0f;                                // the same maximum about the CELL's centre
#endif
    if (uniform) {                                   // one x, y per row segment: |p - c|^2 = dxy^2 + max |z - cz|^2
#pragma unroll
        for (int t = 0; t < SDFK_RLOADS; ++t) {
            const float dx = r.X[t].x - cx, dy = r.Y[t].x - cy;
            const float zm = sd_rawmax(sd_rawmax(sd_abs(r.Z[t].x - cz), sd_abs(r.Z[t].y - cz)),
                                       sd_rawmax(sd_abs(r.Z[t].z - cz), sd_abs(r.Z[t].w - cz)));
            d2 = sd_rawmax(d2, sd_fma(zm, zm, sd_fma(dx, dx, dy * dy)));
#ifdef SDFK_CELLS
            const float ex = r.X[t].x - S.x, ey = r.Y[t].x - S.y;
            const float em = sd_rawmax(sd_rawmax(sd_abs(r.Z[t].x - S.z), sd_abs(r.Z[t].y - S.z)),
                                       sd_rawmax(sd_abs(r.Z[t].z - S.z), sd_abs(r.Z[t].w - S.z)));
            d2s = sd_rawmax(d2s, sd_fma(em, em, sd_fma(ex, ex, ey * ey)));
#endif
        }
    } else {
#pragma unroll
        for (int t = 0; t < SDFK_RLOADS; ++t) {
            const f2 xa = {r.X[t].x, r.X[t].y}, xb = {r.X[t].z, r.X[t].w}, ya = {r.Y[t].x, r.Y[t].y}, yb = {r.Y[t].z, r.Y[t].w};
            const f2 za = {r.Z[t].x, r.Z[t].y}, zb = {r.Z[t].z, r.Z[t].w};
            const f2 ax = xa - cx, ay = ya - cy, az = za - cz, bx = xb - cx, by = yb - cy, bz = zb - cz;
            const f2 da = sd_fma(ax, ax, sd_fma(ay, ay, az * az)), db = sd_fma(bx, bx, sd_fma(by, by, bz * bz));
            d2 = sd_rawmax(d2, sd_rawmax(sd_rawmax(da.x, da.y), sd_rawmax(db.x, db.y)));
#ifdef SDFK_CELLS
            const f2 ex = xa - S.x, ey = ya - S.y, ez = za - S.z, fx = xb - S.x, fy = yb - S.y, fz = zb - S.z;
            const f2 ea = sd_fma(ex, ex, sd_fma(ey, ey, ez * ez)), eb = sd_fma(fx, fx, sd_fma(fy, fy, fz * fz));
            d2s = sd_rawmax(d2s, sd_rawmax(sd_rawmax(ea.x, ea.y), sd_rawmax(eb.x, eb.y)));
#endif
        }
    }
    const float r2 = sdfk_wave_max(d2);
#ifdef SDFK_CELLS
    // inside: max |p - S| <= radius of S, with room for the rounding of the distances (relative 1e-5; S.w < 0: no cell)
    const float rs2 = sdfk_wave_max(d2s);
    if (lane == 0) meta->inside[b] = (S.w > 0.0f && 1.00002f * sqrtf(rs2) <= S.w) ? 1u : 0u;
#endif
    if (lane == 0) {
#ifdef SDFK_FLAT
        meta->bound[b] = make_float4(cx, cz, cy, 1.00001f * sqrtf(r2) + 1e-30f);
#else
        meta->bound[b] = make_float4(cx, cy, cz, 1.00001f * sqrtf(r2) + 1e-30f);
#endif
        meta->uniform[b] = uniform ? 1u : 0u;
#ifdef SDFK_SIMT
#pragma unroll
        for (int w = 0; w < SDFK_NMASK; ++w) meta->mask[w][b] = ~0ull;   // the fold lanes AND their decisions into these
#endif
    }
}
#if defined(SDFK_SIMT) && SDFK_NSUB > 1
// Probe centre `sb` of brick b whose rows each have one x and one y: the sub-brick is rows [r0, r0 + RPS) x points
// [i0, i0 + ZPS) of the window; sphere around the midpoint of its first and last point, radius = the exact maximum
// over its points (read back from the staged coordinates), so any input is bounded correctly — on a regular grid
// 4 rows x 8 points have a quarter of the brick's radius.
static __device__ __forceinline__ float4 sdfk_sub_centre(const sdfk_rowmeta* meta, unsigned b, unsigned sb) {
    constexpr int NZP = 4, NRP = SDFK_NSUB / NZP, RPS = SDFK_RROWS / NRP, ZPS = SDFK_RZ / NZP;
    static_assert(ZPS % 4 == 0 && RPS >= 1, "sub-brick shape");
    int r0 = (int)(sb / NZP) * RPS, r1 = r0 + RPS;
    const int i0 = (int)(sb % NZP) * ZPS;
    if constexpr (NRP == 2) {
        // A brick whose 16 rows come from TWO planes of the grid (1 row block in 32 at 513^3: the last rows of one plane,
        // y near its maximum, and the first rows of the next, y near its minimum) is split where x changes instead of in the
        // middle: each part lies in one plane and is bounded tightly; split in the middle, the part that holds the plane
        // change spans the whole y extent and nothing of the brick could be culled.
        const float x0 = meta->xy[b][0].x;
        if (__builtin_bit_cast(unsigned, x0) != __builtin_bit_cast(unsigned, meta->xy[b][SDFK_RROWS - 1].x)) {
            int s = 1;
            while (s < SDFK_RROWS - 1 && __builtin_bit_cast(unsigned, meta->xy[b][s].x) == __builtin_bit_cast(unsigned, x0)) ++s;
            r0 = sb / NZP ? s : 0;
            r1 = sb / NZP ? SDFK_RROWS : s;
        }
    }
    const float2 pa = meta->xy[b][r0], pe = meta->xy[b][r1 - 1];
    const float za = meta->z[b][r0 * SDFK_RZ + i0], ze = meta->z[b][(r1 - 1) * SDFK_RZ + i0 + ZPS - 1];
    const float cx = 0.5f * (pa.x + pe.x), cy = 0.5f * (pa.y + pe.y), cz = 0.5f * (za + ze);
    float r2 = 0.0f;
#pragma unroll 1
    for (int rr = r0; rr < r1; ++rr) {
        const int r = rr - r0;
        const float2 p = meta->xy[b][r0 + r];
        const float dx = p.x - cx, dy = p.y - cy;
        float zm = 0.0f;
#pragma unroll
        for (int i = 0; i < ZPS; i += 4) {
            const float4 q = *reinterpret_cast<const float4*>(&meta->z[b][(r0 + r) * SDFK_RZ + i0 + i]);
            zm = sd_rawmax(sd_rawmax(zm, sd_abs(q.x - cz)), sd_rawmax(sd_abs(q.y - cz), sd_rawmax(sd_abs(q.z - cz), sd_abs(q.w - cz))));
        }
        r2 = sd_rawmax(r2, sd_fma(zm, zm, sd_fma(dx, dx, dy * dy)));
    }
    const float rho = 1.00001f * sqrtf(r2) + 1e-30f;
#ifdef SDFK_FLAT
    return make_float4(cx, cz, cy, rho);                         // (the staged coordinate is y, xy holds (x, z = 0))
#else
    return make_float4(cx, cy, cz, rho);
#endif
}
#endif

#if defined(SDFK_CHAIN) && !defined(SDFK_CELLS)
// Chain mode, one WAVE per brick: which children run on this brick, from the leaf values at its centre. A hard min (max:
// signs flipped, e_k = +-d_k) is exact, associative and commutative, so the ORDER of the chain does not matter for a
// decision: child k can be dropped wherever some other child j stays below it on the whole brick, and with j = the child
// that is smallest at the centre that is guaranteed by e_k - m >= thr, m = min_j e_j, thr = K rho + margins with
// K = the largest Lipschitz sum of the chain (any pair). No prefix minimum, no "restart" level: one reduction for m, then
// 64 children per step — compare, ballot, and the survivors written as a LIST in index order, so that the evaluation
// never looks at a child it skips and still combines the others in the chain's order. (Tighter than the sequential rule,
// which compares a child with its predecessors only.)
static __device__ __forceinline__ void sdfk_chain_fold(sdfk_rowmeta* meta, int b, int lane) {
    const float4 cc = meta->bound[b];
    const float rho = cc.w, cmag = 1e-6f * (fabsf(cc.x) + fabsf(cc.y) + fabsf(cc.z) + rho);
    constexpr int NW = (SDFK_NLEAF + 63) / 64;
    float m = 3.0e38f;
#pragma unroll 4
    for (int j = 0; j < NW; ++j) {
        const int k = 64 * j + lane;
        if (k < SDFK_NLEAF) m = fminf(m, SDFK_CHAIN_SGN * meta->leafval[k * SDFK_NCEN + b]);
    }
#pragma unroll
    for (int o = 1; o < 64; o <<= 1) m = fminf(m, __shfl_xor(m, o));
    const float thr0 = 1.0001f * SDFK_CHAIN_KMAX * rho + SDFK_CHAIN_KMAX * cmag + 1e-6f * (1.0f + fabsf(m));
    int n_out = 0;
#pragma unroll 1
    for (int j = 0; j < NW; ++j) {
        const int k = 64 * j + lane;
        const bool in = k < SDFK_NLEAF;
        const float e = in ? SDFK_CHAIN_SGN * meta->leafval[k * SDFK_NCEN + b] : 3.0e38f;
        const bool run = in && !(e - m >= thr0 + 1e-6f * fabsf(e));
        const unsigned long long bits = __ballot(run);
        if (run) meta->alist[b][n_out + __builtin_popcountll(bits & ((1ull << lane) - 1ull))] = (unsigned short)k;
        n_out += __builtin_popcountll(bits);
    }
    if (lane == 0) meta->nalive[b] = (unsigned)n_out;
}
#endif

#ifdef SDFK_CELLS
// rows of row block rb plus the cell of brick (rb, window c) and that cell's sphere (wave-uniform; scalar loads)
static __device__ __forceinline__ void sdfk_brick_cell(const sdfk_rowgeom& g, const sdfk_cells& cl, unsigned rb, unsigned c,
                                                       long long& r0, long long& rend, uint2& span, float4& S) {
    unsigned slot, blk;
    sdfk_block_rows(g, rb, r0, rend, &slot, &blk);
    const unsigned sx = slot == 0xffffffffu ? 0u : cl.lv.xoff + slot;
    const unsigned cell = ((sx >> cl.lv.lx) * cl.lv.ncy + (blk >> cl.lv.ly)) * cl.lv.ncz + (c >> cl.lv.lz);
    S = make_float4(0.0f, 0.0f, 0.0f, -1.0f);
    span = make_uint2(0u, SDFK_ALL_ALIVE);
    // (the launch is padded with bricks beyond the last one: their row block does not exist, and neither does a cell for it)
    if (cl.enabled && r0 < rend && cell < cl.ncells) {
        const uint2 sp = cl.span[cell];
        span = make_uint2(__builtin_amdgcn_readfirstlane(sp.x), __builtin_amdgcn_readfirstlane(sp.y));
        const float4 t = cl.sph[cell];
#ifdef SDFK_FLAT
        S = make_float4(t.x, t.z, t.y, t.w);                   // (the registers of phase A hold (x, z, y))
#else
        S = t;
#endif
    }
}
#endif
#if defined(SDFK_CHAIN) && defined(SDFK_CELLS)
// The same decision from the CELL's candidate list: one member per lane, evaluated at the brick's centre on the spot (no
// table of leaf values in LDS) — the first 64 stay in a register, longer lists are evaluated a second time for the
// comparison. A brick that is not inside its cell's sphere, or whose cell has no list, takes every member.
// `sp` (the cell's span) and `first` (this lane's entry of the first batch) were loaded BEFORE the coordinates were waited
// for, so the only memory round trip left between the bounds and the decision is the members' parameters.
static __device__ __forceinline__ void sdfk_chain_fold_cells(sdfk_rowmeta* meta, int b, int lane, const sdfk_cells& cl, uint2 sp,
                                                             unsigned first, const float* __restrict__ PRM,
                                                             const float* __restrict__ TAB) {
    const float4 cc = meta->bound[b];
    const V3T<float> ctr = {cc.x, cc.y, cc.z};
    const float rho = cc.w, cmag = 1e-6f * (fabsf(cc.x) + fabsf(cc.y) + fabsf(cc.z) + rho);
    unsigned off = 0u, cnt = SDFK_NLEAF;
    bool listed = false;
    if (cl.enabled && __builtin_amdgcn_readfirstlane(meta->inside[b]) != 0u && sp.y != SDFK_ALL_ALIVE) {
        off = sp.x; cnt = sp.y; listed = true;
    }
    float m = 3.0e38f, e0 = 3.0e38f;
    unsigned r0 = 0u;
#pragma unroll 1
    for (unsigned j0 = 0u; j0 < cnt; j0 += 64u) {
        const unsigned j = j0 + (unsigned)lane;
        const bool in = j < cnt;
        unsigned rec = 0u;
        if (in) rec = listed ? (j0 == 0u ? first : cl.cand[off + j]) : sdfk_member_record(j);
        float e = 3.0e38f;
        if (in) e = SDFK_CHAIN_SGN * sdfk_leaf_rec<float>(rec, ctr, PRM, TAB);
        if (j0 == 0u) { e0 = e; r0 = rec; }
        m = fminf(m, e);
    }
#pragma unroll
    for (int o = 1; o < 64; o <<= 1) m = fminf(m, __shfl_xor(m, o));
    const float thr0 = 1.0001f * SDFK_CHAIN_KMAX * rho + SDFK_CHAIN_KMAX * cmag + 1e-6f * (1.0f + fabsf(m));
    unsigned n_out = 0u;
#pragma unroll 1
    for (unsigned j0 = 0u; j0 < cnt; j0 += 64u) {
        const unsigned j = j0 + (unsigned)lane;
        const bool in = j < cnt;
        unsigned rec = r0;
        float e = e0;
        if (j0 != 0u) {
            rec = in ? (listed ? cl.cand[off + j] : sdfk_member_record(j)) : 0u;
            e = 3.0e38f;
            if (in) e = SDFK_CHAIN_SGN * sdfk_leaf_rec<float>(rec, ctr, PRM, TAB);
        }
        const bool run = in && !(e - m >= thr0 + 1e-6f * fabsf(e));
        const unsigned long long bits = __ballot(run);
        const unsigned pos = n_out + (unsigned)__builtin_popcountll(bits & ((1ull << lane) - 1ull));
        if (run && pos < SDFK_ALIST_CAP) meta->alist[b][pos] = rec;
        n_out += (unsigned)__builtin_popcountll(bits);
    }
    // more survivors than the list in LDS holds (dense scenes): the brick runs its cell's whole candidate list straight from
    // memory — a superset in the chain's order — and every member only where there is no such list
    if (lane == 0) {
        meta->nalive[b] = n_out <= SDFK_ALIST_CAP ? n_out : (listed ? SDFK_LIST_ALIVE : SDFK_ALL_ALIVE);
        meta->aspan[b] = make_uint2(off, cnt);
    }
}
#endif

// phases A and B of the tile of this workgroup; returns this wave's first brick (row block, window)
#ifdef SDFK_CELLS
#define SDFK_CELLS_PARAM , const sdfk_cells& cl
#define SDFK_CELLS_PASS , cl
#else
#define SDFK_CELLS_PARAM
#define SDFK_CELLS_PASS
#endif
template <typename SRC>
static __device__ __forceinline__ void sdfk_rows_prepare(const float* __restrict__ PRM, const float* __restrict__ TAB,
                                                         const SRC& s, const sdfk_rowgeom& g, sdfk_rowmeta* meta,
                                                         unsigned tile, unsigned& rb0, unsigned& c0 SDFK_CELLS_PARAM) {
    const int lane = sdfk_tx() & 63, wave = __builtin_amdgcn_readfirstlane(sdfk_tx() >> 6);
    const unsigned q0 = tile * SDFK_RNBRICK + wave * SDFK_RWBRICKS;            // first brick of this wave
    rb0 = sdfk_udiv(q0, g.nchunk, g.inv_nchunk);                // (back in an SGPR: what is derived from it stays scalar)
    c0 = q0 - rb0 * g.nchunk;
    unsigned rb = rb0, c = c0;
#if SDFK_RWBRICKS <= 2 && !defined(SDFK_NOHOIST)
    // two-wave workgroups on the north-star grid; with four bricks per wave the registers this takes cost more)
    sdfk_rowregs hregs[SDFK_RWBRICKS];
    bool live[SDFK_RWBRICKS];
#ifdef SDFK_CELLS
    uint2 cspan[SDFK_RWBRICKS];
    unsigned cfirst[SDFK_RWBRICKS];
    float4 csph[SDFK_RWBRICKS];
#endif
#pragma unroll
    for (int j = 0; j < SDFK_RWBRICKS; ++j) {
        long long r0, rend;
#ifdef SDFK_CELLS
        sdfk_brick_cell(g, cl, rb, c, r0, rend, cspan[j], csph[j]);
        cfirst[j] = 0u;                                          // the lane's entry of the list's first batch: in flight with the coordinates
        if (cspan[j].y != SDFK_ALL_ALIVE && (unsigned)lane < cspan[j].y) cfirst[j] = cl.cand[cspan[j].x + (unsigned)lane];
#else
        sdfk_block_rows(g, rb, r0, rend);
#endif
        live[j] = q0 + j < g.nbricks && r0 < rend;               // (blocks of the last plane beyond the slab: nothing)
        if (live[j]) sdfk_rows_load(s, g, r0, rend, c, lane, hregs[j]);
        if (++c == g.nchunk) { c = 0; ++rb; }
    }
#pragma unroll
    for (int j = 0; j < SDFK_RWBRICKS; ++j)
#ifdef SDFK_CELLS
        if (live[j]) sdfk_rows_bounds(hregs[j], lane, meta, wave * SDFK_RWBRICKS + j, csph[j]);
#else
        if (live[j]) sdfk_rows_bounds(hregs[j], lane, meta, wave * SDFK_RWBRICKS + j);
#endif
        else if (lane == 0) { meta->bound[wave * SDFK_RWBRICKS + j] = make_float4(0.0f, 0.0f, 0.0f, 1.0f); meta->uniform[wave * SDFK_RWBRICKS + j] = 0u; }   // (masks: never read)
#else
#ifdef SDFK_CELLS
    bool live[SDFK_RWBRICKS];
    uint2 cspan[SDFK_RWBRICKS];
    unsigned cfirst[SDFK_RWBRICKS];
#endif
#pragma unroll
    for (int j = 0; j < SDFK_RWBRICKS; ++j) {
        long long r0, rend;
#ifdef SDFK_CELLS
        float4 csph;
        sdfk_brick_cell(g, cl, rb, c, r0, rend, cspan[j], csph);
        cfirst[j] = 0u;
        if (cspan[j].y != SDFK_ALL_ALIVE && (unsigned)lane < cspan[j].y) cfirst[j] = cl.cand[cspan[j].x + (unsigned)lane];
        live[j] = q0 + j < g.nbricks && r0 < rend;
#else
        sdfk_block_rows(g, rb, r0, rend);
#endif
#ifdef SDFK_ABLATE_EDGE
        if (q0 + j < g.nbricks && r0 < rend && sdfk_interior(g.L, c)) {
#else
        if (q0 + j < g.nbricks && r0 < rend) {
#endif
            sdfk_rowregs regs;
            sdfk_rows_load(s, g, r0, rend, c, lane, regs);
#ifdef SDFK_CELLS
            sdfk_rows_bounds(regs, lane, meta, wave * SDFK_RWBRICKS + j, csph);
#else
            sdfk_rows_bounds(regs, lane, meta, wave * SDFK_RWBRICKS + j);
#endif
        } else if (lane == 0) {                                   // a dead brick still meets a probe lane: harmless values
            meta->bound[wave * SDFK_RWBRICKS + j] = make_float4(0.0f, 0.0f, 0.0f, 1.0f);
            meta->uniform[wave * SDFK_RWBRICKS + j] = 0u;
        }
        if (++c == g.nchunk) { c = 0; ++rb; }
    }
#endif
    __syncthreads();
#if defined(SDFK_CHAIN) && defined(SDFK_CELLS)
    // every wave folds ITS bricks from their cells' lists: nothing crosses waves any more (no probe centres, no table of
    // leaf values, two barriers fewer than the path below)
#pragma unroll
    for (int j = 0; j < SDFK_RWBRICKS; ++j) {
        const int b = wave * SDFK_RWBRICKS + j;
#ifdef SDFK_ABLATE_PROBE
        if (lane == 0) { meta->alist[b][0] = sdfk_member_record(0u); meta->nalive[b] = live[j] ? 1u : 0u; }
#else
        if (live[j]) sdfk_chain_fold_cells(meta, b, lane, cl, cspan[j], cfirst[j], PRM, TAB);
        else if (lane == 0) meta->nalive[b] = 0u;
#endif
    }
    __syncthreads();
    return;
#endif
#if defined(SDFK_SIMT) && !defined(SDFK_CELLS)
    // lane-parallel probe: probe centres -> every leaf at every centre (all lanes) -> one fold lane per centre ANDs its
    // skip decisions into the brick's mask (a subtree is skipped only if every sub-brick allows it)
    if (sdfk_tx() < SDFK_NCEN) {
        const unsigned b = sdfk_tx() / SDFK_NSUB, sb = sdfk_tx() % SDFK_NSUB;
        float4 cc = meta->bound[b];
#if SDFK_NSUB > 1
        if (meta->uniform[b]) cc = sdfk_sub_centre(meta, b, sb);
#else
        (void)sb;
#endif
        meta->cen[sdfk_tx()] = cc;
    }
    __syncthreads();
#ifndef SDFK_ABLATE_PROBE
    sdfk_probe_leaves(meta->cen, meta->leafval, PRM, TAB);
    __syncthreads();
#ifdef SDFK_CHAIN
#pragma unroll 1
    for (int j = 0; j < SDFK_RWBRICKS; ++j)
        if (q0 + j < g.nbricks) sdfk_chain_fold(meta, wave * SDFK_RWBRICKS + j, lane);
    __syncthreads();
    return;
#else
    if (sdfk_tx() < SDFK_NCEN && tile * SDFK_RNBRICK + sdfk_tx() / SDFK_NSUB < g.nbricks) {
        const float4 cc = meta->cen[sdfk_tx()];
        V3T<float> ctr = {cc.x, cc.y, cc.z};
        unsigned long long mk[SDFK_NMASK];
        sdfk_probe_fold(meta->leafval, sdfk_tx(), ctr, cc.w, PRM, mk);
#pragma unroll
        for (int w = 0; w < SDFK_NMASK; ++w)
            __hip_atomic_fetch_and(&meta->mask[w][sdfk_tx() / SDFK_NSUB], mk[w], __ATOMIC_RELAXED, __HIP_MEMORY_SCOPE_WORKGROUP);
    }
#endif
#else
    if (sdfk_tx() < SDFK_RNBRICK) {
#pragma unroll
        for (int w = 0; w < SDFK_NMASK; ++w) meta->mask[w][sdfk_tx()] = 0ull;
    }
#endif
    __syncthreads();
    return;
#endif
    if (sdfk_tx() < SDFK_RNBRICK && tile * SDFK_RNBRICK + sdfk_tx() < g.nbricks) {
        const float4 bb = meta->bound[sdfk_tx()];
        V3T<float> ctr = {bb.x, bb.y, bb.z};
        unsigned long long mk[SDFK_NMASK];
#pragma unroll
        for (int w = 0; w < SDFK_NMASK; ++w) mk[w] = 0ull;
#if !defined(SDFK_ABLATE_PROBE) && !defined(SDFK_CHAIN)
        sdfk_probe_r(ctr, bb.w, PRM, TAB, mk);
#endif
#pragma unroll
        for (int w = 0; w < SDFK_NMASK; ++w) meta->mask[w][sdfk_tx()] = mk[w];
    }
    __syncthreads();
}

template <typename SRC>
static __device__ __forceinline__ void sdfk_rows_kernel(const float* __restrict__ PRM, const float* __restrict__ TAB,
                                                        const SRC& s, const sdfk_rowgeom& g, float* __restrict__ out,
                                                        unsigned* __restrict__ flags, unsigned thr SDFK_CELLS_PARAM) {
    __shared__ __attribute__((aligned(16))) sdfk_rowmeta meta;
#ifdef SDFK_LDSPAD
    if (g.L == 0xffffffffu) meta.pad[sdfk_tx()] = 1.0f;
#endif
    const int lane = sdfk_tx() & 63, wave = __builtin_amdgcn_readfirstlane(sdfk_tx() >> 6);
    const int lr = lane / SDFK_RLPR;
    const int zq = (lane % SDFK_RLPR) * (2 * SDFK_NP);
#ifndef SDFK_RTILES
#define SDFK_RTILES 1
#endif
#ifndef SDFK_XGROUP
#ifdef SDFK_FLAT                         // flat grids (rows of 16385 points: 513 windows): short runs — the 50-member union at
#define SDFK_XGROUP 4
#else
#define SDFK_XGROUP (SDFK_RNBRICK <= 4 ? 16 : (SDFK_RNBRICK <= 8 ? 8 : 4))    // runs of about 64 bricks: two row blocks at 1025
#endif
#endif
#pragma unroll 1
  for (unsigned tt = 0; tt < SDFK_RTILES; ++tt) {
    // Workgroups go round-robin to the 8 XCDs: an XCD takes runs of SDFK_XGROUP consecutive tiles (the grid is a
    // multiple of 8 * SDFK_XGROUP) instead of every eighth tile, while all XCDs stay in the same neighbourhood of the
    // in all of them (DESIGN 9.1).
    const unsigned xg_t = sdfk_bx() / 8;
    const unsigned tile = (((xg_t / SDFK_XGROUP) * 8 + sdfk_bx() % 8) * SDFK_XGROUP + xg_t % SDFK_XGROUP) * SDFK_RTILES + tt;
    if (tile * SDFK_RNBRICK >= g.nbricks) break;
    if (tt) __syncthreads();
    unsigned rb, c;
    sdfk_rows_prepare(PRM, TAB, s, g, &meta, tile, rb, c SDFK_CELLS_PASS);
    const unsigned q0 = tile * SDFK_RNBRICK + wave * SDFK_RWBRICKS;
#pragma unroll 1
    for (int j = 0; j < SDFK_RWBRICKS; ++j) {
        if (q0 + j >= g.nbricks) break;
        const int b = wave * SDFK_RWBRICKS + j;
        const unsigned k = c;
        long long r0, rend;
        sdfk_block_rows(g, rb, r0, rend);
        if (++c == g.nchunk) { c = 0; ++rb; }
        if (r0 >= rend) continue;
        unsigned mw[2 * SDFK_NMASK];                             // the brick's skip bits as scalar words
#pragma unroll
        for (int w = 0; w < SDFK_NMASK; ++w) {
            const unsigned long long m = meta.mask[w][b];
            mw[2 * w] = __builtin_amdgcn_readfirstlane((unsigned)m);
            mw[2 * w + 1] = __builtin_amdgcn_readfirstlane((unsigned)(m >> 32));
        }
        const bool uniform = __builtin_amdgcn_readfirstlane(meta.uniform[b]) != 0u;
        const bool interior = sdfk_interior(g.L, k);
#ifdef SDFK_ABLATE_EDGE
        if (!interior) continue;
#endif
        const bool live_row = r0 + lr < rend;
        const int dr = live_row ? lr : (int)(rend - 1 - r0);
        long long f;                                              // flat index of this lane's first point
        const int z = sdfk_win_z(r0 + dr, g.L, k, zq, &f);        // its index in the row (edge chunks: may lie outside)
        const int last = (int)g.L - 1;
        V3P P[SDFK_NP];
        f2 res[SDFK_NP];
        // the staged coordinate: z (SDFK_FLAT: y, see sdfk_rows_load)
#ifdef SDFK_FLAT
        SDFK_EACH P[q].y = *reinterpret_cast<const f2*>(&meta.z[b][lr * SDFK_RZ + zq + 2 * q]);
#else
        SDFK_EACH P[q].z = *reinterpret_cast<const f2*>(&meta.z[b][lr * SDFK_RZ + zq + 2 * q]);
#endif
#ifdef SDFK_ABLATE_EVAL
        if (true) {
#ifdef SDFK_FLAT
            SDFK_EACH res[q] = P[q].y + __builtin_bit_cast(float, mw[0] ^ mw[1] ^ mw[2] ^ mw[3]);
#else
            SDFK_EACH res[q] = P[q].z + __builtin_bit_cast(float, mw[0] ^ mw[1] ^ mw[2] ^ mw[3]);
#endif
        } else
#endif
        if (uniform) {
            const float2 xy = meta.xy[b][lr];
#ifdef SDFK_FLAT
            SDFK_EACH { P[q].x = sp<f2>(xy.x); P[q].z = sp<f2>(xy.y); }      // (x, 0)
#else
            SDFK_EACH { P[q].x = sp<f2>(xy.x); P[q].y = sp<f2>(xy.y); }
#endif
#ifndef SDFK_CHAIN
            sdfk_rows_culled<true>(xy.x, xy.y, P, mw, PRM, TAB, res);
#endif
        } else {                                                  // the other coordinates of every point again (L2-resident)
#pragma unroll
            for (int q = 0; q < SDFK_NP; q += 2) {
                float4 X, Y, Z;
                sdfk_rows_fetch(s, g, r0, dr, z + 2 * q, interior, X, Y, Z);
                P[q].x = {X.x, X.y};
                P[q + 1].x = {X.z, X.w};
#ifdef SDFK_FLAT
                P[q].z = {Z.x, Z.y};
                P[q + 1].z = {Z.z, Z.w};
#else
                P[q].y = {Y.x, Y.y};
                P[q + 1].y = {Y.z, Y.w};
#endif
            }
#ifndef SDFK_CHAIN
            sdfk_rows_culled<false>(0.0f, 0.0f, P, mw, PRM, TAB, res);
#endif
        }
#ifdef SDFK_CHAIN
        {   // The children on the brick's list, in order; the first one starts the accumulator. Looked up one by one — kind of
            // the child, base of its parameters, then the parameters: three dependent scalar loads per child — the evaluation
            // the next SDFK_CHUNK children lane-parallel — a lane per (child, parameter) — into LDS, and then evaluates them
            // from there: the latency is paid once per chunk.
#ifdef SDFK_CELLS
            // (more survivors than the list holds — nalive = ALL —: every member, in order, straight from its index)
            const unsigned nal = __builtin_amdgcn_readfirstlane(meta.nalive[b]);
            const bool all_alive = nal == SDFK_ALL_ALIVE, list_alive = nal == SDFK_LIST_ALIVE;
            const unsigned aoff = __builtin_amdgcn_readfirstlane(meta.aspan[b].x);
            const unsigned cnt = all_alive ? (unsigned)SDFK_NLEAF : (list_alive ? __builtin_amdgcn_readfirstlane(meta.aspan[b].y) : nal);
#define SDFK_AREC(i) (all_alive ? sdfk_member_record(i) : (list_alive ? cl.cand[aoff + (i)] : meta.alist[b][i]))
#else
            const unsigned cnt = __builtin_amdgcn_readfirstlane(meta.nalive[b]);
#define SDFK_AREC(i) sdfk_member_record((unsigned)meta.alist[b][i])
#endif
            f2 acc[SDFK_NP];
#if SDFK_CHAIN_STAGED
            if (cnt <= SDFK_STAGE_MIN)
#endif
            {
                // one or two survivors (the 50-child flat union: 1.06 per brick): staging costs more than it hides, and
                // parameters in SGPRs beat parameters read back from LDS — straight from the table
#pragma unroll 1
                for (unsigned i = 0; i < cnt; ++i) {
                    const unsigned rec = __builtin_amdgcn_readfirstlane(SDFK_AREC(i));
                    f2 val[SDFK_NP];
                    SDFK_EACH val[q] = sdfk_leaf_rec<f2>(rec, P[q], PRM, TAB);
                    if (i == 0u) { SDFK_EACH acc[q] = val[q]; }
                    else { SDFK_EACH acc[q] = SDFK_CHAIN_CMB(acc[q], val[q], PRM); }
                }
            }
#if SDFK_CHAIN_STAGED
            else
#pragma unroll 1
            for (unsigned c0 = 0; c0 < cnt; c0 += SDFK_CHUNK) {
                const unsigned nc = cnt - c0 < SDFK_CHUNK ? cnt - c0 : SDFK_CHUNK;
                __builtin_amdgcn_fence(__ATOMIC_RELEASE, "wavefront");      // (the previous chunk has been read)
                __builtin_amdgcn_wave_barrier();
#pragma unroll 1
                for (unsigned it = (unsigned)lane; it < nc * SDFK_NPLMAX; it += 64u) {
                    const unsigned ch = it / SDFK_NPLMAX, w = it - ch * SDFK_NPLMAX;
                    const unsigned rec = SDFK_AREC(c0 + ch);
                    const unsigned at = (rec & 0xffffffu) + w;
                    meta.cprm[b][ch][w] = PRM[at < SDFK_NPARAMS ? at : SDFK_NPARAMS - 1u];
                    if (w == 0u) meta.cgrp[b][ch] = rec >> 24;
                }
                __builtin_amdgcn_fence(__ATOMIC_RELEASE, "wavefront");
                __builtin_amdgcn_wave_barrier();
                __builtin_amdgcn_fence(__ATOMIC_ACQUIRE, "wavefront");
#pragma unroll 1
                for (unsigned i = 0; i < nc; ++i) {
                    const unsigned grp = __builtin_amdgcn_readfirstlane(meta.cgrp[b][i]);
                    const float* cp = &meta.cprm[b][i][0];
                    f2 val[SDFK_NP];
                    SDFK_EACH val[q] = sdfk_leaf_at<f2>(grp, P[q], cp, TAB);
                    if (c0 + i == 0u) { SDFK_EACH acc[q] = val[q]; }
                    else { SDFK_EACH acc[q] = SDFK_CHAIN_CMB(acc[q], val[q], PRM); }
                }
            }
#endif
            SDFK_EACH res[q] = sdfk_chain_tail<f2>(acc[q], P[q], PRM, TAB);
#if defined(SDFK_DEBUG_NALIVE) && defined(SDFK_CELLS)
            // test aid: instead of the field, how the brick ran — survivors on its list; 100000 + entries when it ran its cell's
            // whole list (more survivors than SDFK_ALIST_CAP); -1 when it ran every member
            SDFK_EACH res[q] = sp<f2>(all_alive ? -1.0f : (list_alive ? 100000.0f + (float)cnt : (float)cnt));
#endif
        }
#endif
#ifdef SDFK_FLAGS                                                  // (the flag-writing build) one bit per point instead of the field
        {
            // BRICK-TILED layout: the word of (row r, window k) is flags[(brick * 16 + r % 16)], so the 64 lanes of the
            // wave — lane = 4 * row + octet of the window — write the brick's 64 bytes as ONE contiguous store, and every
            // (row, window) slot belongs to one brick, also where two rows share a flat window: no atomics (a linear bit
            // string needs an atomic OR in the edge windows and 16 partial-line stores per brick). The compaction
            unsigned bits = 0u;
            SDFK_EACH bits |= ((sdfk_sel_key(res[q].x) <= thr ? 1u : 0u) | (sdfk_sel_key(res[q].y) <= thr ? 2u : 0u)) << (2 * q);
            if (!interior) {                                       // an edge window: only the points of this row
                unsigned ok = 0u;
                SDFK_EACH {
                    if (z + 2 * q >= 0 && z + 2 * q <= last) ok |= 1u << (2 * q);
                    if (z + 2 * q + 1 >= 0 && z + 2 * q + 1 <= last) ok |= 2u << (2 * q);
                }
// ... 157 lines not shown
    }
#pragma unroll 4
    for (unsigned j0 = 64u * SDFK_CELL_NB; j0 < cnt; j0 += 64u) {
        const unsigned j = j0 + (unsigned)lane;
        if (j < cnt) m = fminf(m, SDFK_CHAIN_SGN * sdfk_leaf_rec<float>(listed ? cp.cand[off + j] : sdfk_member_record(j), c, PRM, TAB));
    }
#pragma unroll
    for (int o = 1; o < 64; o <<= 1) m = fminf(m, __shfl_xor(m, o));
    const float thr0 = 1.0001f * SDFK_CHAIN_KMAX * rho + SDFK_CHAIN_KMAX * cmag + 1e-6f * (1.0f + fabsf(m));
    unsigned total = 0u;
#pragma unroll
    for (int bt = 0; bt < SDFK_CELL_NB; ++bt)
        if (64u * bt < cnt) total += (unsigned)__builtin_popcountll(__ballot(64u * bt + (unsigned)lane < cnt && !(ev[bt] - m >= thr0 + 1e-6f * fabsf(ev[bt]))));
#pragma unroll 4
    for (unsigned j0 = 64u * SDFK_CELL_NB; j0 < cnt; j0 += 64u) {
        const unsigned j = j0 + (unsigned)lane;
        bool run = false;
        if (j < cnt) {
            const float e = SDFK_CHAIN_SGN * sdfk_leaf_rec<float>(listed ? cp.cand[off + j] : sdfk_member_record(j), c, PRM, TAB);
            run = !(e - m >= thr0 + 1e-6f * fabsf(e));
        }
        total += (unsigned)__builtin_popcountll(__ballot(run));
    }
    // per microsecond and address), so the pool is cut into SDFK_POOL_SHARDS shards with a head each, dealt by cell index
    unsigned at = 0u;
    const unsigned shard = cell & (SDFK_POOL_SHARDS - 1u);
    if (lane == 0) at = atomicAdd(cp.head + 16u * shard, total);
    at = __shfl(at, 0);
    if (at > cp.shard_cap || total > cp.shard_cap - at) {       // the shard is full: bricks of this cell probe every member
        if (lane == 0) cp.span[cell] = make_uint2(0u, SDFK_ALL_ALIVE);
        return;
    }
    at += cp.base + shard * cp.shard_cap;
    unsigned n_out = 0u;
#pragma unroll
    for (int bt = 0; bt < SDFK_CELL_NB; ++bt)
        if (64u * bt < cnt) {
            const bool run = 64u * bt + (unsigned)lane < cnt && !(ev[bt] - m >= thr0 + 1e-6f * fabsf(ev[bt]));
            const unsigned long long bits = __ballot(run);
            if (run) cp.cand[at + n_out + (unsigned)__builtin_popcountll(bits & ((1ull << lane) - 1ull))] = rv[bt];
            n_out += (unsigned)__builtin_popcountll(bits);
        }
#pragma unroll 4
    for (unsigned j0 = 64u * SDFK_CELL_NB; j0 < cnt; j0 += 64u) {
        const unsigned j = j0 + (unsigned)lane;
        bool run = false;
        unsigned rec = 0u;
        if (j < cnt) {
            rec = listed ? cp.cand[off + j] : sdfk_member_record(j);
            const float e = SDFK_CHAIN_SGN * sdfk_leaf_rec<float>(rec, c, PRM, TAB);
            run = !(e - m >= thr0 + 1e-6f * fabsf(e));
        }
        const unsigned long long bits = __ballot(run);
        if (run) cp.cand[at + n_out + (unsigned)__builtin_popcountll(bits & ((1ull << lane) - 1ull))] = rec;
        n_out += (unsigned)__builtin_popcountll(bits);
    }
    if (lane == 0) cp.span[cell] = make_uint2(at, total);
}
#else
#define SDFK_CELLS_KARG
#endif
)SDFKR";
static const char kRowsArray[] = R"SDFKR(
extern "C" __global__ __launch_bounds__(64 * SDFK_RWAVES) SDFK_ROWS_ATTR void sdfk_spec_r(
    const float* __restrict__ PRM, const float* __restrict__ TAB, const float* __restrict__ co, long long stride,
    sdfk_rowgeom g, float* __restrict__ out, unsigned* __restrict__ flags, unsigned thr SDFK_CELLS_KARG) {
    const SrcArray s = {co, stride};
    sdfk_rows_kernel(PRM, TAB, s, g, out, flags, thr SDFK_CELLS_PASS);
}
#ifdef SDFK_CELLS
extern "C" __global__ __launch_bounds__(256) void sdfk_spec_cells(
    const float* __restrict__ PRM, const float* __restrict__ TAB, const float* __restrict__ co, long long stride,
    sdfk_rowgeom g, sdfk_cellpass cp) {
    const SrcArray s = {co, stride};
    sdfk_cells_kernel(PRM, TAB, s, g, cp);
}
#endif
)SDFKR";
static const char kRowsGrid[] = R"SDFKR(
// the same on a regular grid expanded from three per-axis tables (no coordinate array: 4 B/point); the slab
// starts at a row boundary and out[0] is its first point
extern "C" __global__ __launch_bounds__(64 * SDFK_RWAVES) void sdfk_spec_rg(
    const float* __restrict__ PRM, const float* __restrict__ TAB, SrcGrid s, sdfk_rowgeom g, float* __restrict__ out,
    unsigned* __restrict__ flags, unsigned thr SDFK_CELLS_KARG) {
    sdfk_rows_kernel(PRM, TAB, s, g, out, flags, thr SDFK_CELLS_PASS);
}
#ifdef SDFK_CELLS
extern "C" __global__ __launch_bounds__(256) void sdfk_spec_cellsg(
    const float* __restrict__ PRM, const float* __restrict__ TAB, SrcGrid s, sdfk_rowgeom g, sdfk_cellpass cp) {
    sdfk_cells_kernel(PRM, TAB, s, g, cp);
}
#endif
)SDFKR";
static const char kRowsMask[] = R"SDFKR(
// test aid: the skip masks (two 64-bit words per brick: sites 0-31, 32-63; bit 2k = first operand of site k
// skipped, bit 2k+1 = second) followed by the "uniform rows" flag in a third word
extern "C" __global__ __launch_bounds__(64 * SDFK_RWAVES) void sdfk_spec_rmask(
    const float* __restrict__ PRM, const float* __restrict__ TAB, const float* __restrict__ co, long long stride,
    sdfk_rowgeom g, unsigned long long* __restrict__ masks) {
    __shared__ __attribute__((aligned(16))) sdfk_rowmeta meta;
    const SrcArray s = {co, stride};
    unsigned rb, c;
    sdfk_rows_prepare(PRM, TAB, s, g, &meta, sdfk_bx(), rb, c);
    const unsigned q = sdfk_bx() * SDFK_RNBRICK + sdfk_tx();
    if (sdfk_tx() < SDFK_RNBRICK && q < g.nbricks) {
        masks[3ull * q] = meta.mask[0][sdfk_tx()];
        masks[3ull * q + 1] = meta.mask[1][sdfk_tx()];
        masks[3ull * q + 2] = meta.uniform[sdfk_tx()];
    }
}
)SDFKR";

namespace {

struct Gen {
    const sdfk_opinfo* ops;
    int n_ops;
    const uint32_t* code;
    size_t n_instr;
    const std::vector<sdfk_cullsite>* sites;
    std::string s;
    bool rows = false;

    std::vector<int> root_slot;
    int n_root = 0;
    void find_roots() {
        root_slot.assign(n_instr, -1);
        bool c0_intact = true;
        for (size_t i = 0; i < n_instr; ++i) {
            const uint32_t w = code[2 * i];
            const unsigned op = w & 255u, a = (w >> 8) & 255u, b = (w >> 16) & 255u;
            if ((int)op >= n_ops) continue;
            if (ops[op].kind != SDFK_KIND_C_C) continue;
            if (!strcmp(ops[op].name, "XFORM") && b == 0 && c0_intact && n_root < 64) root_slot[i] = n_root++;
            if (a == 0) c0_intact = false;
        }
    }

    void instr_x(size_t i, const char* indent, int mode) {
        const int r = root_slot.empty() ? -1 : root_slot[i];
        if (r < 0 || mode == 0 || (rows && mode == 1)) {
            instr(i, indent, rows && mode == 2);
            return;
        }
        char buf[1400];
        const uint32_t w = code[2 * i], poff = code[2 * i + 1];
        const unsigned a = (w >> 8) & 255u;
        if (rows) {
            snprintf(buf, sizeof buf,
                     "%sif constexpr (ZRUN) {\n"
                     "#ifdef SDFK_FLAT\n"
                     "%s  const V3T<float> bs = op_xform_base_x(X, PRM + %u);\n"
                     "%s  const V3P bp = {sp<f2>(bs.x), sp<f2>(bs.y), sp<f2>(bs.z)};\n"
                     "%s  SDFK_EACH C_%u[q] = op_xform_y(bp, C_0[q].y, PRM + %u);\n"
                     "#else\n"
                     "%s  const V3T<float> bs = op_xform_base(X, Y, PRM + %u);\n"
                     "%s  const V3P bp = {sp<f2>(bs.x), sp<f2>(bs.y), sp<f2>(bs.z)};\n"
                     "%s  SDFK_EACH C_%u[q] = op_xform_z(bp, C_0[q].z, PRM + %u);\n"
                     "#endif\n"
                     "%s} else { SDFK_EACH C_%u[q] = op_xform(C_0[q], PRM + %u, TAB, 0); }\n",
                     indent, indent, poff, indent, indent, a, poff, indent, poff, indent, indent, a, poff, indent, a, poff);
        } else if (mode == 1) {
            snprintf(buf, sizeof buf,
                     "%s{ const V3T<float> bs = op_xform_base(C_0.x, C_0.y, PRM + %u); bases[%d] = bs.x; bases[%d] = bs.y; "
                     "bases[%d] = bs.z;\n%s  C_%u = op_xform_z(bs, C_0.z, PRM + %u); }\n",
                     indent, poff, 3 * r, 3 * r + 1, 3 * r + 2, indent, a, poff);
        } else {
            snprintf(buf, sizeof buf,
// ... 850 lines not shown
            g.s += "\n#define SDFK_NP 4\n#define SDFK_EACH _Pragma(\"unroll\") for (int q = 0; q < SDFK_NP; ++q)\n"
                   "#define SDFK_NMASK 2\n"
                   "#define SDFK_SIMT 1\n#define SDFK_NSUB 1\n"
                   "#ifndef SDFK_CELLS_MIN_LEAVES\n#define SDFK_CELLS_MIN_LEAVES 64\n#endif\n"
                   "#if !defined(SDFK_NO_CELLS) && SDFK_NLEAF > SDFK_CELLS_MIN_LEAVES\n#define SDFK_CELLS 1\n#endif\n"
                   "#ifndef SDFK_LEAF_UNROLL\n#define SDFK_LEAF_UNROLL _Pragma(\"unroll 4\")\n#endif\n";
            g.s += kSimtGeometry;
            g.emit_probe_leaves(g.leaves.size() >= 128, true);
            g.s += kRowsKernel;
            if (all || flavour == SDFK_FL_ROWS_ARRAY || flavour == SDFK_FL_ROWS2D_ARRAY) g.s += kRowsArray;
            if (all || flavour == SDFK_FL_ROWS_GRID || flavour == SDFK_FL_ROWS2D_GRID) g.s += kRowsGrid;
        }
        return g.s;
    }
    if (plain) {
        g.s += "\ntemplate <typename T> static __device__ __forceinline__ T sdfk_point(V3T<T> C_0, "
               "const float* __restrict__ PRM, const float* __restrict__ TAB, const float* __restrict__ AUX, "
               "long long AUXS) {\n";
        g.declare("V3T<T>", "T", false);
        for (size_t i = 0; i < n_instr; ++i) g.instr(i, "    ");
        snprintf(buf, sizeof buf, "    return V_%d;\n}\n", result_reg);
        g.s += buf;
        g.s += kWrappers;
        if (all || flavour == SDFK_FL_PLAIN_ARRAY) g.s += kWrappersArray;
        if (all || flavour == SDFK_FL_PLAIN_GRID) g.s += kWrappersGrid;
    }
    if (tile || rowk) g.s += kWaveHelpers;
    if (tile) {
        std::vector<size_t> order(sites.size());
        for (size_t i = 0; i < order.size(); ++i) order[i] = i;
        std::stable_sort(order.begin(), order.end(), [&](size_t x, size_t y) {
            return sites[x].comb - sites[x].a0 > sites[y].comb - sites[y].a0;
        });
        order.resize(std::min<size_t>(order.size(), 31));
        std::sort(order.begin(), order.end());
        std::vector<sdfk_cullsite> flat;
        for (size_t i : order) flat.push_back(sites[i]);
        g.sites = &flat;
        g.find_roots();
        snprintf(buf, sizeof buf, "\n#define SDFK_NROOT %d\n", g.n_root > 0 ? g.n_root : 1);
        g.s += buf;
        g.emit_probe();
        g.emit_culled(result_reg);
        g.s += kTileKernel;
        if (all || flavour == SDFK_FL_TILE_ARRAY) g.s += kTileArray;
        if (all || flavour == SDFK_FL_TILE_GRID) g.s += kTileGrid;
        if (all || flavour == SDFK_FL_TILE_MASK) g.s += kTileMask;
        g.sites = &sites;
    }
    if (rowk) {
        g.rows = true;
        g.root_slot.clear();
        g.n_root = 0;
        g.find_roots();
        if (flat) g.s += "\n#define SDFK_FLAT 1\n";
        g.s += "\n#define SDFK_NP 4\n#define SDFK_EACH _Pragma(\"unroll\") for (int q = 0; q < SDFK_NP; ++q)\n";
        {
            char nm[64];
            snprintf(nm, sizeof nm, "#define SDFK_NMASK %zu\n", std::max<size_t>(2, (sites.size() + 31) / 32));
            g.s += nm;
        }
        g.s += "#ifndef SDFK_CHAIN_LOOP_MIN\n#define SDFK_CHAIN_LOOP_MIN 100000   // chains of at least this many sites run as a loop over the levels that survive\n#endif\n"
               "// the even bits of x, packed into the low 32 bits (wave-uniform: scalar unit)\n"
               "static __device__ __forceinline__ unsigned long long sdfk_even_bits(unsigned long long x) {\n"
               "    x &= 0x5555555555555555ull;\n"
               "    x = (x | (x >> 1)) & 0x3333333333333333ull;\n"
               "    x = (x | (x >> 2)) & 0x0f0f0f0f0f0f0f0full;\n"
               "    x = (x | (x >> 4)) & 0x00ff00ff00ff00ffull;\n"
               "    x = (x | (x >> 8)) & 0x0000ffff0000ffffull;\n"
               "    x = (x | (x >> 16)) & 0x00000000ffffffffull;\n"
               "    return x;\n}\n";
        g.simt = g.analyse_leaves();
        if (g.simt) {
            char def[160];
            snprintf(def, sizeof def, "\n#ifndef SDFK_NOSIMT\n#define SDFK_SIMT 1\n#endif\n#define SDFK_NLEAF %zu\n", g.leaves.size());
            g.s += def;
            g.s += kSimtGeometry;
            g.emit_groups();
            g.emit_probe_leaves();
            g.emit_probe_fold();
        }
        g.emit_probe();
        g.emit_rows_culled(result_reg);
        g.s += kRowsKernel;
        if (all || flavour == SDFK_FL_ROWS_ARRAY || flavour == SDFK_FL_ROWS2D_ARRAY) g.s += kRowsArray;
        if (all || flavour == SDFK_FL_ROWS_GRID || flavour == SDFK_FL_ROWS2D_GRID) g.s += kRowsGrid;
        if (all || flavour == SDFK_FL_ROWS_MASK) g.s += kRowsMask;
    }
    return g.s;
}
```

### aegolius_amd/csrc/sdfk_occupancy.inc

```
#include "sdfk_occdev.h"

template <int NC, int NV, typename SRC>
__global__ __launch_bounds__(SDFK_OCC_BLOCK) void sdfk_occ_interp_kernel(const uint2* __restrict__ code, int n_instr,
                                                                        const float* __restrict__ prm,
                                                                        const float* __restrict__ tab, int result_reg, SRC src,
                                                                        sdfk_occgrid grid, float* __restrict__ out) {
    const SdfkInterpField<NC, NV> field = {code, n_instr, prm, tab, result_reg};
    sdfk_occ_sample(src, field, grid, out);
}

#define SDFK_OCC_RUN 1024
#define SDFK_OCC_PARTIALS 4096

struct sdfk_occclass {
    const float* __restrict__ ax0;
    const float* __restrict__ ax1;
    const float* __restrict__ ax2;
    const float* __restrict__ hw0;
    const float* __restrict__ hw1;
    const float* __restrict__ hw2;
    unsigned n1, n2;
    long long first, count;
    float level, lip;
    unsigned level_key;
// ... 147 lines not shown
            if (x) (void)hipEventDestroy(x);
    }
};

extern "C" int sdfk_eval_grid_occupancy(sdfk_program* p, const float* ax0, int64_t n0, const float* ax1, int64_t n1,
                                        const float* ax2, int64_t n2, const float* sub0, const float* sub1, const float* sub2,
                                        const float* hw0, const float* hw1, const float* hw2, int samples, float level,
                                        float lipschitz, float* d_fraction, void* d_scratch, int64_t slab_cells,
                                        int64_t* inside_samples, int64_t* near_cells, float* pass_ms, void* stream_, int mode) {
    const std::string w = "sdfk_eval_grid_occupancy";
    if (!p) return fail(-1, "null program");
    if (!ax0 || !ax1 || !ax2 || !sub0 || !sub1 || !sub2 || !hw0 || !hw1 || !hw2) return fail(-1, w + ": null table");
    if (n0 < 1 || n1 < 1 || n2 < 1 || n1 > 0x7fffffff || n2 > 0x7fffffff || n0 > (1LL << 40))
        return fail(-1, w + ": axis sizes from 1 to 2^31 - 1");
    if (samples != 1 && samples != 2 && samples != 4 && samples != 8) return fail(-1, w + ": samples per axis: 1, 2, 4 or 8");
    if (occ_is_nan(level)) return fail(-1, w + ": the level is NaN");
    if (occ_is_nan(lipschitz) || lipschitz < 0.0f) return fail(-1, w + ": the Lipschitz bound must not be negative or NaN");
    if (!d_fraction || !d_scratch) return fail(-1, w + ": null output or scratch pointer");
    if (!inside_samples || !near_cells) return fail(-1, w + ": null statistics pointer");
    if (mode < SDFK_MODE_AUTO || mode > SDFK_MODE_NOCULL) return fail(-1, w + ": unknown mode");
    int bad = -1;
    const int chk = sdfk_program_rays_check(p, &bad);
    if (chk) return fail(chk < 0 ? chk : -3, w + ": " + g_err);
    if (mode == SDFK_MODE_AUTO) mode = g_default_mode;
    const bool skip = occ_is_finite(lipschitz) && mode != SDFK_MODE_NOCULL;

    const unsigned k0 = n0 > 1 ? samples : 1, k1 = n1 > 1 ? samples : 1, k2 = n2 > 1 ? samples : 1;
    auto lg = [](unsigned k) { return k == 8 ? 3u : k == 4 ? 2u : k == 2 ? 1u : 0u; };
    const unsigned K = k0 * k1 * k2;
    const int64_t total_cells = n0 * n1 * n2;
    const int64_t slab = occ_slab_cells(n0, n1, n2, slab_cells);

    hipStream_t stream = (hipStream_t)stream_;
    int device = 0;
    HIPCHK(hipGetDevice(&device));
    DevState* d = nullptr;
    int rc = ensure_resident(p, device, stream, &d);
    if (rc) return rc;

    AxisTables axes, extra;
    SrcGrid g;
    rc = upload_axes(ax0, n0, ax1, n1, ax2, n2, stream, &axes, &g, 0);
    if (rc) return rc;
    const size_t s0 = (size_t)n0 * k0, s1 = (size_t)n1 * k1, s2 = (size_t)n2 * k2;
    HIPCHK(hipMalloc(&extra.d, (s0 + s1 + s2 + (size_t)(n0 + n1 + n2)) * sizeof(float)));
    float* d_sub[3] = {extra.d, extra.d + s0, extra.d + s0 + s1};
    float* d_hw[3] = {extra.d + s0 + s1 + s2, extra.d + s0 + s1 + s2 + n0, extra.d + s0 + s1 + s2 + n0 + n1};
    HIPCHK(hipMemcpyAsync(d_sub[0], sub0, s0 * sizeof(float), hipMemcpyHostToDevice, stream));
    HIPCHK(hipMemcpyAsync(d_sub[1], sub1, s1 * sizeof(float), hipMemcpyHostToDevice, stream));
    HIPCHK(hipMemcpyAsync(d_sub[2], sub2, s2 * sizeof(float), hipMemcpyHostToDevice, stream));
    HIPCHK(hipMemcpyAsync(d_hw[0], hw0, (size_t)n0 * sizeof(float), hipMemcpyHostToDevice, stream));
    HIPCHK(hipMemcpyAsync(d_hw[1], hw1, (size_t)n1 * sizeof(float), hipMemcpyHostToDevice, stream));
    HIPCHK(hipMemcpyAsync(d_hw[2], hw2, (size_t)n2 * sizeof(float), hipMemcpyHostToDevice, stream));

    char* scratch = (char*)d_scratch;
    unsigned long long* d_partial = (unsigned long long*)scratch;
    unsigned long long* d_blk = (unsigned long long*)(scratch + SDFK_OCC_PARTIALS * 8);
    char* rest = scratch + SDFK_OCC_PARTIALS * 8 + occ_align((size_t)(occ_runs(slab) + 1) * 8);
    float* d_centre = (float*)rest;
    unsigned* d_list = (unsigned*)(rest + occ_align((size_t)slab * 4));

    OccEvents ev;
    if (pass_ms) {
        for (hipEvent_t& x : ev.e) HIPCHK(hipEventCreate(&x));
        pass_ms[0] = pass_ms[1] = pass_ms[2] = 0.0f;
    }
    sdfk_occgrid G = {d_sub[0], d_sub[1], d_sub[2], (unsigned)n1, (unsigned)n2, k1, k2, k0, lg(k1), lg(k2), K,
                      lg(k0) + lg(k1) + lg(k2), 1.0f / (float)K, sdfk_sel_key(level), total_cells < (1LL << 32) ? 1u : 0u, 0};
    sdfk_occclass C = {g.ax0, g.ax1, g.ax2, d_hw[0], d_hw[1], d_hw[2], (unsigned)n1, (unsigned)n2, 0, 0, level, lipschitz,
                       sdfk_sel_key(level)};
    const float* prm = d->d_params;
    const float* tab = d->d_tables;
    const int n_instr = (int)(p->code.size() / 2);
    const unsigned per_wave = K >= 64u ? 1u : 64u / K;
    int64_t near_total = 0;

    for (int64_t first = 0; first < total_cells; first += slab) {
        const int64_t cells = std::min(slab, total_cells - first);
        float* out = d_fraction + first;
        unsigned long long n_entries = (unsigned long long)cells;
        if (pass_ms) HIPCHK(hipEventRecord(ev.e[0], stream));
        if (skip) {
            g.start = first;
            rc = run(p, nullptr, &g, cells, d_centre, stream, mode, true);
            if (rc) return rc;
            if (pass_ms) HIPCHK(hipEventRecord(ev.e[1], stream));
            C.first = first;
            C.count = cells;
            const long long runs = occ_runs(cells);
            const unsigned blocks = (unsigned)((runs + SDFK_OCC_BLOCK / 64 - 1) / (SDFK_OCC_BLOCK / 64));
            hipLaunchKernelGGL(sdfk_occ_classify_kernel<false>, dim3(blocks), dim3(SDFK_OCC_BLOCK), 0, stream,
                               (const float*)d_centre, C, out, d_list, d_blk);
            hipLaunchKernelGGL(sdfk_select_scan_kernel, dim3(1), dim3(1024), 0, stream, d_blk, runs);
            hipLaunchKernelGGL(sdfk_occ_classify_kernel<true>, dim3(blocks), dim3(SDFK_OCC_BLOCK), 0, stream,
                               (const float*)d_centre, C, out, d_list, d_blk);
            HIPCHK(hipGetLastError());
            unsigned long long h = 0;
            HIPCHK(hipMemcpyAsync(&h, d_blk + runs, sizeof h, hipMemcpyDeviceToHost, stream));
            HIPCHK(hipStreamSynchronize(stream));
            if (h > (unsigned long long)cells) return fail(-2, w + ": the list of near cells is longer than the slab");
            n_entries = h;
        } else if (pass_ms) {
            HIPCHK(hipEventRecord(ev.e[1], stream));
        }
        if (pass_ms) HIPCHK(hipEventRecord(ev.e[2], stream));
        near_total += (int64_t)n_entries;
        if (n_entries) {
            G.first = first;
            const unsigned long long waves = (n_entries + per_wave - 1) / per_wave;
            const unsigned blocks = (unsigned)((waves + SDFK_OCC_BLOCK / 64 - 1) / (SDFK_OCC_BLOCK / 64));
            std::shared_ptr<SpecModule> sk;
            if (mode != SDFK_MODE_INTERPRET) {
                static const bool async_jit = [] { const char* e = getenv("SDFK_ASYNC_JIT"); return !(e && e[0] == '0'); }();
                const bool wait = mode != SDFK_MODE_AUTO || !p->interp_ok || !async_jit;
                std::string err;
                sk = get_module(p, device, SDFK_FL_OCCUPANCY, wait, &err);
                if (sk && sk->failed) {
                    if (mode != SDFK_MODE_AUTO || !p->interp_ok)
                        return fail(-3, "specialised occupancy kernel unavailable: " + err);
                    sk.reset();
                }
            }
            if (!sk && !p->interp_ok)
                return fail(-4, "program needs more registers than the interpreter kernel has (use the specialised mode)");
            SdfkOccList src_list = {d_list, n_entries};
            SdfkOccAll src_all = {n_entries};
            if (sk) {
                void* src = skip ? (void*)&src_list : (void*)&src_all;
                void* args[] = {&prm, &tab, src, &G, &out};
                HIPCHK(hipModuleLaunchKernel(sk->fn[skip ? 0 : 1], blocks, 1, 1, SDFK_OCC_BLOCK, 1, 1, 0, stream, args, nullptr));
            } else {
                auto launch = [&](auto src) {
                    using SRC = decltype(src);
                    if (p->interp_small)
                        hipLaunchKernelGGL((sdfk_occ_interp_kernel<SDFK_NC_SMALL, SDFK_NV_SMALL, SRC>), dim3(blocks),
                                           dim3(SDFK_OCC_BLOCK), 0, stream, d->d_code, n_instr, prm, tab, p->result_reg, src, G, out);
                    else
                        hipLaunchKernelGGL((sdfk_occ_interp_kernel<SDFK_NC, SDFK_NV, SRC>), dim3(blocks), dim3(SDFK_OCC_BLOCK), 0,
                                           stream, d->d_code, n_instr, prm, tab, p->result_reg, src, G, out);
                };
                if (skip) launch(src_list);
                else launch(src_all);
                HIPCHK(hipGetLastError());
            }
        }
        if (pass_ms) {
            HIPCHK(hipEventRecord(ev.e[3], stream));
            HIPCHK(hipEventSynchronize(ev.e[3]));
            for (int k = 0; k < 3; ++k) {
                float ms = 0.0f;
                HIPCHK(hipEventElapsedTime(&ms, ev.e[k], ev.e[k + 1]));
                pass_ms[k] += ms;
            }
        }
    }
    hipLaunchKernelGGL(sdfk_occ_total_kernel, dim3(SDFK_OCC_PARTIALS / 4), dim3(256), 0, stream, (const float*)d_fraction,
                       (long long)total_cells, (float)K, d_partial);
    HIPCHK(hipGetLastError());
    std::vector<unsigned long long> partial(SDFK_OCC_PARTIALS);
    HIPCHK(hipMemcpyAsync(partial.data(), d_partial, partial.size() * 8, hipMemcpyDeviceToHost, stream));
    HIPCHK(hipStreamSynchronize(stream));
    unsigned long long inside = 0;
    for (unsigned long long v : partial) inside += v;
    *inside_samples = (int64_t)inside;
    *near_cells = near_total;
    return 0;
}
// ... 1 lines not shown
```

### include/sdfk.h

```cpp
#ifndef SDFK_H
#define SDFK_H

#include <stddef.h>
#include <stdint.h>

#ifdef __cplusplus
extern "C" {
#endif

#define SDFK_ABI_VERSION 1

#define SDFK_MODE_AUTO 0
#define SDFK_MODE_INTERPRET 1
#define SDFK_MODE_SPECIALIZED 2
#define SDFK_MODE_NOCULL 3

typedef struct sdfk_program sdfk_program;

int sdfk_abi_version(void);
int sdfk_device_count(void);
const char* sdfk_last_error(void);

sdfk_program* sdfk_program_create(const uint32_t* code, size_t n_instr, const float* params, size_t n_params,
                                  const float* tables, size_t n_tables, int result_reg);
void sdfk_program_destroy(sdfk_program* prog);
int sdfk_program_set_params(sdfk_program* prog, const float* params, size_t n_params);
int sdfk_program_set_cull(sdfk_program* prog, const uint32_t* sites, size_t n_sites, const float* k);
int sdfk_program_chain_members(const sdfk_program* prog);
const char* sdfk_program_source(sdfk_program* prog);
int sdfk_program_compile_check(sdfk_program* prog, size_t* code_size);
#define SDFK_FLAVOUR_PLAIN_ARRAY 0
#define SDFK_FLAVOUR_PLAIN_GRID 1
#define SDFK_FLAVOUR_TILE_ARRAY 2
#define SDFK_FLAVOUR_TILE_GRID 3
#define SDFK_FLAVOUR_TILE_MASK 4
#define SDFK_FLAVOUR_ROWS_ARRAY 5
#define SDFK_FLAVOUR_ROWS_GRID 6
#define SDFK_FLAVOUR_ROWS_MASK 7
#define SDFK_FLAVOUR_ROWS2D_ARRAY 8
#define SDFK_FLAVOUR_ROWS2D_GRID 9
#define SDFK_FLAVOUR_RAYS 10
#define SDFK_FLAVOUR_OCCUPANCY 11
#define SDFK_FLAVOUR_FLAGS 0x100
#define SDFK_FLAVOUR_XY 0x200
int sdfk_program_compile_flavour(sdfk_program* prog, int flavour, size_t* code_size, double* seconds);
void sdfk_debug_cells_stats(int enable, long long* out8);
void sdfk_debug_rays_stats(int enable, long long* out8);
int sdfk_debug_compile_external(sdfk_program* prog, int flavour, size_t* code_size);
void sdfk_jit_drain(void);
void sdfk_jit_cancel(void);
void sdfk_debug_jit_stats(int64_t* builds, double* seconds);
void sdfk_debug_set_rtc_defs(const char* defs);

int sdfk_eval_device(sdfk_program* prog, const float* d_co, int64_t n, int64_t row_stride, float* d_out,
                     void* stream, int mode);
int sdfk_eval_device_rows(sdfk_program* prog, const float* d_co, int64_t n, int64_t row_stride, int64_t row_len,
                          float* d_out, void* stream, int mode);
int sdfk_eval_device_rows3d(sdfk_program* prog, const float* d_co, int64_t n, int64_t row_stride, int64_t row_len,
                            int64_t plane_rows, int64_t first_row_in_plane, float* d_out, void* stream, int mode);
int sdfk_eval_device_rows2d(sdfk_program* prog, const float* d_co, int64_t n, int64_t row_stride, int64_t row_len,
                            float* d_out, void* stream, int mode);
int sdfk_eval_device_rows2d_xy(sdfk_program* prog, const float* d_xy, int64_t n, int64_t row_stride, int64_t row_len,
                               float* d_out, void* stream, int mode);
int sdfk_eval_host(sdfk_program* prog, const void* co, int co_dtype, int64_t n, int64_t row_stride, float* out,
                   int device, int mode);
int sdfk_eval_host_resident(sdfk_program* prog, const void* co, int co_dtype, int64_t n, int64_t row_stride,
                            float* d_out, int device, int mode);
int sdfk_eval_grid(sdfk_program* prog, const float* ax0, int64_t n0, const float* ax1, int64_t n1, const float* ax2,
                   int64_t n2, int64_t start, int64_t count, float* d_out, void* stream, int mode);
int sdfk_eval_grid_host(sdfk_program* prog, const float* ax0, int64_t n0, const float* ax1, int64_t n1,
                        const float* ax2, int64_t n2, int64_t start, int64_t count, float* out, int device, int mode);
int sdfk_eval_grid_sharded(sdfk_program* prog, const float* ax0, int64_t n0, const float* ax1, int64_t n1,
                           const float* ax2, int64_t n2, int n_shards, const int* devices, float* out, int mode);
int sdfk_eval_grid_sharded_device(sdfk_program* prog, const float* ax0, int64_t n0, const float* ax1, int64_t n1,
                                  const float* ax2, int64_t n2, int n_shards, const int* devices, int gather_device,
                                  float* d_full, int mode);
void sdfk_set_default_mode(int mode);
int sdfk_debug_brick_masks(sdfk_program* prog, const float* d_co, int64_t n, int64_t row_stride, uint64_t* d_masks,
                           void* stream);
int sdfk_debug_row_masks(sdfk_program* prog, const float* d_co, int64_t n, int64_t row_stride, int64_t row_len,
                         uint64_t* d_masks, int64_t* n_bricks, int* brick_rows, void* stream);

int sdfk_eval_device_aux(sdfk_program* prog, const float* d_co, int64_t n, int64_t row_stride, const float* d_aux,
                         int n_aux, int64_t aux_stride, float* d_out, void* stream, int mode);
int sdfk_eval_grid_aux(sdfk_program* prog, const float* ax0, int64_t n0, const float* ax1, int64_t n1, const float* ax2,
                       int64_t n2, int64_t start, int64_t count, const float* d_aux, int n_aux, int64_t aux_stride,
                       float* d_out, void* stream, int mode);
int sdfk_field_min(const float* d_field, int64_t n, float* out_min, void* stream);
int sdfk_grid_box_average(float* d_field, int64_t n0, int64_t n1, int64_t n2, int k0, int k1, int k2, int iterations,
                          void* d_scratch, void* stream);
int sdfk_grid_edge_detect(float* d_field, int64_t n0, int64_t n1, int64_t n2, void* d_scratch, void* stream);
int sdfk_grid_signed(float* d_field, int64_t n0, int64_t n1, int64_t n2, float sep_min, int crop, void* d_scratch,
                     void* stream);
int sdfk_debug_box_variant(int64_t n0, int64_t n1, int64_t n2, int k0, int k1, int k2, int* out8);
int sdfk_grid_boundary_mask(const float* d_field, int64_t n, float sep_min, unsigned char* d_mask, void* stream);
int sdfk_grid_signed_slab(float* d_slab, int64_t plane0, int64_t planes, const unsigned char* d_mask, int64_t n0, int64_t n1,
                          int64_t n2, int crop, void* d_scratch, void* stream);

size_t sdfk_field_select_scratch(int64_t n);
int sdfk_field_select_finish(int64_t n, int64_t count, int64_t* d_index, int64_t capacity, void* d_scratch, void* stream);

size_t sdfk_eval_select_scratch(int64_t n, int64_t row_len);
int sdfk_eval_device_select(sdfk_program* prog, const float* d_co, int64_t n, int64_t row_stride, int64_t row_len, int flat,
                            float threshold, int64_t* d_index, int64_t capacity, int64_t* count, void* d_scratch,
                            void* stream, int mode);
int sdfk_eval_grid_select(sdfk_program* prog, const float* ax0, int64_t n0, const float* ax1, int64_t n1, const float* ax2,
                          int64_t n2, int64_t start, int64_t count_points, float threshold, int64_t* d_index,
                          int64_t capacity, int64_t* count, void* d_scratch, void* stream, int mode);
int sdfk_eval_select_finish(sdfk_program* prog, int64_t n, int64_t row_len, int mode, int64_t count, int64_t* d_index,
                            int64_t capacity, void* d_scratch, void* stream);
int sdfk_field_select(const float* d_field, int64_t n, float threshold, int64_t* d_index, int64_t capacity,
                      int64_t* count, void* d_scratch, void* stream);
int sdfk_field_gradient(const float* d_field, int64_t n0, int64_t n1, int64_t n2, int ncomp, int normalize,
                        float* d_vec, int64_t row_stride, void* stream);

int sdfk_field_crossings_2d(const float* d_uu, const float* d_ww, int64_t n0, int64_t n1, int64_t n2, double w, double d,
                            double thr, signed char* d_sign, void* stream);
int sdfk_lcwg_eval(int variant, const float* d_uu, const float* d_ww, int64_t n0, int64_t n1, int64_t n2, double w, double d,
                   int sign_kind, double sign_value, const void* d_sign, float* d_vec, int64_t row_stride, void* stream);
int sdfk_lcwg_old_eval(int variant, const float* d_r, int64_t r_stride, const float* d_uu, int64_t n, double w, double d,
                       float* d_vec, int64_t row_stride, void* stream);

typedef struct {
    int32_t op;
    int32_t src[2];
    float imm[4];
} sdfk_vec_instr;
int sdfk_vec_eval_device(const sdfk_vec_instr* prog, int n_instr, const float* d_p, int64_t n, int64_t p_stride,
                         const float* d_streams, int n_streams, int64_t stream_stride, int out_kind, float* d_out,
                         int64_t out_stride, void* stream);
void sdfk_vec_set_interpret(int on);
const char* sdfk_vec_source(const sdfk_vec_instr* prog, int n_instr, int n_streams, int out_kind);
int sdfk_vec_compile_check(const sdfk_vec_instr* prog, int n_instr, int n_streams, int out_kind, size_t* code_size);
int sdfk_vec_eval_host(const sdfk_vec_instr* prog, int n_instr, const void* p, int p_dtype, int64_t n, const float* ax0,
                       int64_t n0, const float* ax1, int64_t n1, const float* ax2, int64_t n2, const float* streams,
// ... 99 lines not shown
```

Measured before the change: 372,000.

## Load axis-table grid coordinates directly into registers in row-block kernel

```diff
diff --git a/aegolius_amd/_engine.py b/aegolius_amd/_engine.py
--- a/aegolius_amd/_engine.py
+++ b/aegolius_amd/_engine.py
@@ -38,6 +38,8 @@
     "sdfk_jit_drain": (None, []),
     "sdfk_jit_cancel": (None, []),
     "sdfk_debug_set_rtc_defs": (None, [_c.c_char_p]),
+    "sdfk_debug_grid_rowsplit": (_int, [_i64, _c.c_uint32, _c.c_uint32, _c.POINTER(_c.c_uint64), _c.POINTER(_c.c_uint32),
+                                 _c.POINTER(_c.c_uint32)]),
     "sdfk_eval_device": (_int, [_vp, _vp, _i64, _i64, _vp, _vp, _int]),
     "sdfk_eval_device_rows": (_int, [_vp, _vp, _i64, _i64, _i64, _vp, _vp, _int]),
     "sdfk_eval_device_rows2d": (_int, [_vp, _vp, _i64, _i64, _i64, _vp, _vp, _int]),
diff --git a/aegolius_amd/csrc/sdfk.hip b/aegolius_amd/csrc/sdfk.hip
--- a/aegolius_amd/csrc/sdfk.hip
+++ b/aegolius_amd/csrc/sdfk.hip
@@ -1091,10 +1091,12 @@
     return e;
 }
 static std::string flavour_key(const sdfk_program* p, int flavour, int rwb, int with_flags = 0) {
-    return p->key + "|f" + std::to_string(flavour) + ((with_flags & 1) ? "s" : "") + ((with_flags & 2) ? "x" : "") + "|" + rtc_option_key(rwb);
+    return p->key + "|f" + std::to_string(flavour) + ((with_flags & 1) ? "s" : "") + ((with_flags & 2) ? "x" : "") +
+           ((with_flags & 4) ? "g" : "") + "|" + rtc_option_key(rwb);
 }
 static std::string flavour_source(const sdfk_program* p, int flavour, int with_flags = 0) {
     return std::string((with_flags & 1) ? "#define SDFK_FLAGS 1\n" : "") + ((with_flags & 2) ? "#define SDFK_XY 1\n" : "") +
+           ((with_flags & 4) ? "#define SDFK_GRID_STAGED 1\n" : "") +
            sdfk_generate_source(g_ops, SDFK_OP_COUNT, p->code.data(), p->code.size() / 2, p->result_reg, p->sites, flavour,
                                 &p->sites_all);
 }
@@ -1438,7 +1440,7 @@
 static int run(sdfk_program* p, const SrcArray* arr, const SrcGrid* grid, long long n, float* d_out, void* stream_,
                int mode, bool vec_ok, long long row_len = 0, const float* aux = nullptr, long long aux_stride = 0,
                bool flat = false, long long plane_rows = 0, long long plane_phase = 0, unsigned* d_flags = nullptr,
-               unsigned thr_key = 0, bool xy = false) {
+               unsigned thr_key = 0, bool xy = false, bool z_monotone = false) {
     if (!p) return fail(-1, "null program");
     if (n < 0) return fail(-1, "negative point count");
     if (p->n_aux > 0 && (!aux || aux_stride < n))
@@ -1497,7 +1499,8 @@
         static const bool async_jit = [] { const char* e = getenv("SDFK_ASYNC_JIT"); return !(e && e[0] == '0'); }();
         const bool wait = mode != SDFK_MODE_AUTO || !p->interp_ok || !async_jit;
         std::string err;
-        sk = get_module(p, device, flavour, wait, &err, (d_flags ? 1 : 0) | (xy ? 2 : 0));
+        const bool staged = flavour == SDFK_FL_ROWS_GRID && !d_flags && !p->chain_mode && !(z_monotone && rg.R <= 0x7fffffffLL);
+        sk = get_module(p, device, flavour, wait, &err, (d_flags ? 1 : 0) | (xy ? 2 : 0) | (staged ? 4 : 0));
         if (sk && sk->failed) {
             if (mode == SDFK_MODE_SPECIALIZED || !p->interp_ok)
                 return fail(-3, "specialised kernel unavailable: " + err);
@@ -1541,7 +1544,8 @@
                     rc = prepare_cells(p, d, sk->fn[1], rg, src, 1, prm, tab, stream, &cells);
                     if (rc) return rc;
                 }
-                void* args[] = {&prm, &tab, &g, &rg, &d_out, &d_flags, &thr_key, &cells};
+                sdfk_rowbase gb = sdfk_grid_rowbase(rg.row0, grid->n1);
+                void* args[] = {&prm, &tab, &g, &rg, &d_out, &d_flags, &thr_key, p->chain_mode ? (void*)&cells : (void*)&gb};
                 HIPCHK(hipModuleLaunchKernel(sk->fn[0], tiles, 1, 1, rthreads, 1, 1, 0, stream, args, nullptr));
             }
             return 0;
@@ -1762,6 +1766,7 @@
 
 struct AxisTables {
     float* d = nullptr;
+    bool z_monotone = false;
     ~AxisTables() {
         if (d) (void)hipFree(d);
     }
@@ -1775,12 +1780,36 @@
     HIPCHK(hipMemcpyAsync(t->d, ax0, (size_t)n0 * sizeof(float), hipMemcpyHostToDevice, stream));
     HIPCHK(hipMemcpyAsync(t->d + n0, ax1, (size_t)n1 * sizeof(float), hipMemcpyHostToDevice, stream));
     HIPCHK(hipMemcpyAsync(t->d + n0 + n1, ax2, (size_t)n2 * sizeof(float), hipMemcpyHostToDevice, stream));
+    bool up = true, down = true;
+    for (int64_t i = 0; i < n2; ++i) {
+        if (!std::isfinite(ax2[i])) up = down = false;
+        if (i > 0 && !(ax2[i - 1] <= ax2[i])) up = false;
+        if (i > 0 && !(ax2[i - 1] >= ax2[i])) down = false;
+    }
+    t->z_monotone = up || down;
     g->ax0 = t->d;
     g->ax1 = t->d + n0;
     g->ax2 = t->d + n0 + n1;
     g->n1 = (unsigned)n1;
     g->n2 = (unsigned)n2;
     g->start = start;
+    return 0;
+}
+
+static int run_grid(sdfk_program* p, const SrcGrid& g, const AxisTables& t, long long n, float* d_out, void* stream, int mode,
+                    bool vec_ok, const float* aux = nullptr, long long aux_stride = 0) {
+    return run(p, nullptr, &g, n, d_out, stream, mode, vec_ok, 0, aux, aux_stride, false, 0, 0, nullptr, 0, false, t.z_monotone);
+}
+
+extern "C" int sdfk_debug_grid_rowsplit(int64_t row0, uint32_t n1, uint32_t r, uint64_t* ix, uint32_t* iy, uint32_t* inv_n1) {
+    if (row0 < 0 || n1 < 1 || n1 > 0x7fffffffu || r > 0x7fffffffu || !ix || !iy) return fail(-1, "sdfk_debug_grid_rowsplit: bad arguments");
+    const sdfk_rowbase b = sdfk_grid_rowbase((long long)row0, n1);
+    unsigned long long x;
+    unsigned y;
+    sdfk_grid_rowsplit(b, n1, r, x, y);
+    *ix = x;
+    *iy = y;
+    if (inv_n1) *inv_n1 = b.inv_n1;
     return 0;
 }
 
@@ -1793,7 +1822,7 @@
     SrcGrid g;
     int rc = upload_axes(ax0, n0, ax1, n1, ax2, n2, (hipStream_t)stream, &t, &g, start);
     if (rc) return rc;
-    rc = run(p, nullptr, &g, count, d_out, stream, mode, aligned16(d_out));
+    rc = run_grid(p, g, t, count, d_out, stream, mode, aligned16(d_out));
     if (rc) return rc;
     HIPCHK(hipStreamSynchronize((hipStream_t)stream));
     return 0;
@@ -1809,7 +1838,7 @@
     SrcGrid g;
     int rc = upload_axes(ax0, n0, ax1, n1, ax2, n2, (hipStream_t)stream, &t, &g, start);
     if (rc) return rc;
-    rc = run(p, nullptr, &g, count, d_out, stream, mode, aligned16(d_out), 0, d_aux, aux_stride);
+    rc = run_grid(p, g, t, count, d_out, stream, mode, aligned16(d_out), d_aux, aux_stride);
     if (rc) return rc;
     HIPCHK(hipStreamSynchronize((hipStream_t)stream));
     return 0;
@@ -1834,7 +1863,7 @@
     for (int64_t s = 0; s < count && rc == 0; s += chunk) {
         const int64_t m = std::min(chunk, count - s);
         g.start = start + s;
-        rc = run(p, nullptr, &g, m, d_out, nullptr, mode, true);
+        rc = run_grid(p, g, t, m, d_out, nullptr, mode, true);
         if (rc == 0 && hipMemcpy(out + s, d_out, (size_t)m * sizeof(float), hipMemcpyDeviceToHost) != hipSuccess)
             rc = fail(-6, "sdfk_eval_grid_host: device-to-host copy failed");
     }
diff --git a/aegolius_amd/csrc/sdfk_access.h b/aegolius_amd/csrc/sdfk_access.h
--- a/aegolius_amd/csrc/sdfk_access.h
+++ b/aegolius_amd/csrc/sdfk_access.h
@@ -14,6 +14,27 @@
     unsigned n1, n2;
     long long start;
 };
+
+struct sdfk_rowbase {
+    unsigned long long ix0;
+    unsigned iy0, inv_n1;
+};
+static __host__ __device__ __forceinline__ sdfk_rowbase sdfk_grid_rowbase(long long row0, unsigned n1) {
+    sdfk_rowbase b;
+    b.ix0 = (unsigned long long)row0 / n1;
+    b.iy0 = (unsigned)((unsigned long long)row0 - b.ix0 * n1);
+    const unsigned long long inv = (1ull << 32) / n1;
+    b.inv_n1 = inv > 0xffffffffull ? 0xffffffffu : (unsigned)inv;
+    return b;
+}
+static __host__ __device__ __forceinline__ void sdfk_grid_rowsplit(const sdfk_rowbase& b, unsigned n1, unsigned r,
+                                                                   unsigned long long& ix, unsigned& iy) {
+    unsigned q = (unsigned)(((unsigned long long)r * b.inv_n1) >> 32);
+    while (r - q * n1 >= n1) ++q;
+    ix = b.ix0 + q;
+    iy = b.iy0 + (r - q * n1);
+    if (iy >= n1) { iy -= n1; ++ix; }
+}
 
 typedef float sdfk_f4 __attribute__((ext_vector_type(4)));
 static __device__ __forceinline__ float4 sdfk_stream_load4(const float* p) {
diff --git a/aegolius_amd/csrc/sdfk_codegen.cpp b/aegolius_amd/csrc/sdfk_codegen.cpp
--- a/aegolius_amd/csrc/sdfk_codegen.cpp
+++ b/aegolius_amd/csrc/sdfk_codegen.cpp
@@ -671,8 +671,15 @@
 #define SDFK_ALL_ALIVE 0xffffffffu
 #define SDFK_LIST_ALIVE 0xfffffffeu
 #endif
+#if defined(SDFK_GRID_DIRECT) && (defined(SDFK_CHAIN) || defined(SDFK_CELLS) || defined(SDFK_FLAT) || defined(SDFK_FLAGS) || defined(SDFK_XY))
+#error "SDFK_GRID_DIRECT: field-writing row blocks of a 3-D grid only"
+#endif
 struct sdfk_rowmeta {
+#ifdef SDFK_GRID_DIRECT
+    int zs[SDFK_RNBRICK][SDFK_RROWS];           // index in its row of the first point of the window, per row of the brick
+#else
     float z[SDFK_RNBRICK][SDFK_RBRICK];         // [row of the brick][point of the window]
+#endif
     float2 xy[SDFK_RNBRICK][SDFK_RROWS];
     float4 bound[SDFK_RNBRICK];
     unsigned long long mask[SDFK_NMASK][SDFK_RNBRICK];   // two bits per site: SDFK_NMASK x 32 sites (2 words up to 64 sites)
@@ -857,6 +864,7 @@
 #else
 #define SDFK_CELL_ARG
 #endif
+#ifndef SDFK_GRID_DIRECT                         // (the staged path: sdfk_direct_* below replace it on axis tables)
 static __device__ __forceinline__ void sdfk_rows_bounds(const sdfk_rowregs& r, int lane, sdfk_rowmeta* meta, int b SDFK_CELL_ARG) {
 #ifdef SDFK_ABLATE_BOUNDS
     *reinterpret_cast<float4*>(&meta->z[b][(lane >> 3) * SDFK_RZ + 4 * (lane & 7)]) = r.Z[0];
@@ -949,7 +957,8 @@
 #endif
     }
 }
-#if defined(SDFK_SIMT) && SDFK_NSUB > 1
+#endif
+#if defined(SDFK_SIMT) && SDFK_NSUB > 1 && !defined(SDFK_GRID_DIRECT)
 // Probe centre `sb` of brick b whose rows each have one x and one y: the sub-brick is rows [r0, r0 + RPS) x points
 // [i0, i0 + ZPS) of the window; sphere around the midpoint of its first and last point, radius = the exact maximum
 // over its points (read back from the staged coordinates), so any input is bounded correctly — on a regular grid
@@ -998,6 +1007,94 @@
 }
 #endif
 
+#ifdef SDFK_GRID_DIRECT
+// ---- Row blocks of a grid that is given as three axis tables (sdfk_spec_rg, field-writing build, 3-D grid) ----------
+// The array path above discovers the structure of its data: it loads in the array-load layout, stages z in LDS for the
+// evaluation layout, and tests that every row has one x and one y. Here that structure is known — row r of the slab is
+// (ax0[ix], ax1[iy]) x ax2[0 .. L) — so a lane loads, before the first barrier and for every brick of its wave, exactly
+// what it evaluates: the 2 * SDFK_NP points of ITS row from ax2 and that row's x and y, and keeps them in registers.
+// "Uniform" is a compile-time fact. LDS keeps the 16 row heads of a brick and the index of each row's window start;
+// the probe lanes bound a sub-brick from those: max |z - cz| over the index range its rows cover (the rows of a brick
+// are skewed against each other by L mod 32 points; the union range, clamped like the loads, is a superset) is taken at
+// the ends of the range — the host launches this build only for a monotone, finite ax2 and the staged one otherwise
+// (sdfk.hip: run). As everywhere, the sphere only decides what may be skipped: the field's bits do not depend on it.
+struct sdfk_gridregs {                           // what a lane keeps of ONE brick between the loads and phase C
+    f2 z[SDFK_NP];                               // z of its 2 * SDFK_NP points
+    float2 xy;                                   // x, y of its row
+};
+// loads of one live brick (r0, rend, k wave-uniform); zs = index in the row of the window's first point
+static __device__ __forceinline__ void sdfk_direct_load(const SrcGrid& s, const sdfk_rowgeom& g, const sdfk_rowbase& gb,
+                                                        long long r0, long long rend, unsigned k, int lane,
+                                                        sdfk_gridregs& r, int& zs) {
+    const int lr = lane / SDFK_RLPR, zq = (lane % SDFK_RLPR) * (2 * SDFK_NP);
+    const int nrow = (int)(rend - r0 < (long long)SDFK_RROWS ? rend - r0 : (long long)SDFK_RROWS);   // 1 .. 16 rows
+    const int dr = lr < nrow ? lr : nrow - 1;                     // rows past the block's end: its last row again
+    unsigned long long ix;
+    unsigned iy;
+    sdfk_grid_rowsplit(gb, s.n1, (unsigned)r0, ix, iy);           // scalar unit: once per brick
+    iy += (unsigned)dr;                                           // a block may hold rows of two planes, of several with
+    while (iy >= s.n1) { iy -= s.n1; ++ix; }                      // n1 < 16
+    r.xy = make_float2(s.ax0[ix], s.ax1[iy]);
+    long long f;
+    const int z = sdfk_win_z(r0 + dr, g.L, k, zq, &f);
+    zs = z - zq;
+    const bool interior = sdfk_interior(g.L, k);
+#pragma unroll
+    for (int q = 0; q < SDFK_NP; q += 2) {
+        const float4 Z = sdfk_win_quad(s.ax2, z + 2 * q, (int)g.L - 1, interior);
+        r.z[q] = {Z.x, Z.y};
+        r.z[q + 1] = {Z.z, Z.w};
+    }
+}
+// Probe centre `sb` of NSUB of live brick b: rows [r0, r1) x points [i0, i0 + ZPS) of the window, as sdfk_sub_centre
+// cuts them (a brick of two planes is split where x changes), bounded from the row heads and the ends of the z range
+template <int NSUB>
+static __device__ __forceinline__ float4 sdfk_direct_centre(const sdfk_rowmeta* meta, const float* __restrict__ ax2, int last,
+                                                            unsigned b, unsigned sb) {
+    constexpr int NZP = NSUB >= 4 ? 4 : 1, NRP = NSUB / NZP, RPS = SDFK_RROWS / NRP, ZPS = SDFK_RZ / NZP;
+    static_assert(RPS >= 1 && NRP * RPS == SDFK_RROWS && NZP * ZPS == SDFK_RZ, "sub-brick shape");
+    int r0 = (int)(sb / NZP) * RPS, r1 = r0 + RPS;
+    const int i0 = (int)(sb % NZP) * ZPS;
+    if constexpr (NRP == 2) {
+        const float x0 = meta->xy[b][0].x;
+        if (__builtin_bit_cast(unsigned, x0) != __builtin_bit_cast(unsigned, meta->xy[b][SDFK_RROWS - 1].x)) {
+            int s = 1;
+            while (s < SDFK_RROWS - 1 && __builtin_bit_cast(unsigned, meta->xy[b][s].x) == __builtin_bit_cast(unsigned, x0)) ++s;
+            r0 = sb / NZP ? s : 0;
+            r1 = sb / NZP ? SDFK_RROWS : s;
+        }
+    }
+    const float2 pa = meta->xy[b][r0], pe = meta->xy[b][r1 - 1];
+    const float cx = 0.5f * (pa.x + pe.x), cy = 0.5f * (pa.y + pe.y);
+    int zlo = 0x7fffffff, zhi = -0x7fffffff;
+    float d2 = 0.0f;
+#pragma unroll 1
+    for (int rr = r0; rr < r1; ++rr) {
+        const float2 p = meta->xy[b][rr];
+        const int zz = meta->zs[b][rr];
+        const float dx = p.x - cx, dy = p.y - cy;
+        d2 = sd_rawmax(d2, sd_fma(dx, dx, dy * dy));
+        zlo = min(zlo, zz);
+        zhi = max(zhi, zz);
+    }
+    zlo = min(max(zlo + i0, 0), last);                             // (edge windows: the loads clamp the same way)
+    zhi = min(max(zhi + i0 + ZPS - 1, 0), last);
+    const float za = ax2[zlo], ze = ax2[zhi];
+    const float cz = 0.5f * (za + ze);
+    const float zm = sd_rawmax(sd_abs(za - cz), sd_abs(ze - cz));
+    return make_float4(cx, cy, cz, 1.00001f * sqrtf(sd_fma(zm, zm, d2)) + 1e-30f);
+}
+#define SDFK_DIRECT_PARAM , const sdfk_rowbase& gb, sdfk_gridregs (&gr)[SDFK_RWBRICKS]
+#define SDFK_DIRECT_PASS , gb, gr
+#define SDFK_DIRECT_KARG , sdfk_rowbase gb
+#define SDFK_DIRECT_KPASS , gb
+#else
+#define SDFK_DIRECT_PARAM
+#define SDFK_DIRECT_PASS
+#define SDFK_DIRECT_KARG
+#define SDFK_DIRECT_KPASS
+#endif
+
 #if defined(SDFK_CHAIN) && !defined(SDFK_CELLS)
 // Chain mode, one WAVE per brick: which children run on this brick, from the leaf values at its centre. A hard min (max:
 // signs flipped, e_k = +-d_k) is exact, associative and commutative, so the ORDER of the chain does not matter for a
@@ -1129,13 +1226,55 @@
 template <typename SRC>
 static __device__ __forceinline__ void sdfk_rows_prepare(const float* __restrict__ PRM, const float* __restrict__ TAB,
                                                          const SRC& s, const sdfk_rowgeom& g, sdfk_rowmeta* meta,
-                                                         unsigned tile, unsigned& rb0, unsigned& c0 SDFK_CELLS_PARAM) {
+                                                         unsigned tile, unsigned& rb0, unsigned& c0 SDFK_CELLS_PARAM
+                                                         SDFK_DIRECT_PARAM) {
     const int lane = sdfk_tx() & 63, wave = __builtin_amdgcn_readfirstlane(sdfk_tx() >> 6);
     const unsigned q0 = tile * SDFK_RNBRICK + wave * SDFK_RWBRICKS;            // first brick of this wave
     rb0 = sdfk_udiv(q0, g.nchunk, g.inv_nchunk);                // (back in an SGPR: what is derived from it stays scalar)
     c0 = q0 - rb0 * g.nchunk;
     unsigned rb = rb0, c = c0;
-#if SDFK_RWBRICKS <= 2 && !defined(SDFK_NOHOIST)
+#ifdef SDFK_GRID_DIRECT
+    // all of the wave's loads are in flight before the first one is used; a dead brick (beyond the slab: the launch is
+    // padded) touches no table and leaves harmless values for the probe lane it still meets
+    // (the rows of every brick first: sdfk_udiv is a call that waits for the loads in flight)
+    bool live[SDFK_RWBRICKS];
+    int zs[SDFK_RWBRICKS];
+    long long r0[SDFK_RWBRICKS], rend[SDFK_RWBRICKS];
+    unsigned kk[SDFK_RWBRICKS];
+#pragma unroll
+    for (int j = 0; j < SDFK_RWBRICKS; ++j) {
+        sdfk_block_rows(g, rb, r0[j], rend[j]);
+        live[j] = q0 + j < g.nbricks && r0[j] < rend[j];
+        kk[j] = c;
+        if (++c == g.nchunk) { c = 0; ++rb; }
+    }
+#pragma unroll
+    for (int j = 0; j < SDFK_RWBRICKS; ++j) {
+        if (live[j]) {
+            sdfk_direct_load(s, g, gb, r0[j], rend[j], kk[j], lane, gr[j], zs[j]);
+        } else {
+            SDFK_EACH gr[j].z[q] = sp<f2>(0.0f);
+            gr[j].xy = make_float2(0.0f, 0.0f);
+            zs[j] = 0;
+        }
+    }
+#pragma unroll
+    for (int j = 0; j < SDFK_RWBRICKS; ++j) {
+        const int b = wave * SDFK_RWBRICKS + j;
+        if (live[j] && lane % SDFK_RLPR == 0) {
+            meta->xy[b][lane / SDFK_RLPR] = gr[j].xy;
+            meta->zs[b][lane / SDFK_RLPR] = zs[j];
+        }
+        if (lane == 0) {
+            meta->bound[b] = make_float4(0.0f, 0.0f, 0.0f, 1.0f);
+            meta->uniform[b] = live[j] ? 1u : 0u;                 // here: "live" — a probe lane bounds only such bricks
+#ifdef SDFK_SIMT
+#pragma unroll
+            for (int w = 0; w < SDFK_NMASK; ++w) meta->mask[w][b] = ~0ull;   // the fold lanes AND their decisions into these
+#endif
+        }
+    }
+#elif SDFK_RWBRICKS <= 2 && !defined(SDFK_NOHOIST)
     // two-wave workgroups on the north-star grid; with four bricks per wave the registers this takes cost more)
     sdfk_rowregs hregs[SDFK_RWBRICKS];
     bool live[SDFK_RWBRICKS];
@@ -1226,7 +1365,11 @@
     if (sdfk_tx() < SDFK_NCEN) {
         const unsigned b = sdfk_tx() / SDFK_NSUB, sb = sdfk_tx() % SDFK_NSUB;
         float4 cc = meta->bound[b];
-#if SDFK_NSUB > 1
+#ifdef SDFK_GRID_DIRECT
+#ifndef SDFK_ABLATE_BOUNDS
+        if (meta->uniform[b]) cc = sdfk_direct_centre<SDFK_NSUB>(meta, s.ax2, (int)g.L - 1, b, sb);
+#endif
+#elif SDFK_NSUB > 1
         if (meta->uniform[b]) cc = sdfk_sub_centre(meta, b, sb);
 #else
         (void)sb;
@@ -1264,7 +1407,12 @@
     return;
 #endif
     if (sdfk_tx() < SDFK_RNBRICK && tile * SDFK_RNBRICK + sdfk_tx() < g.nbricks) {
+#if defined(SDFK_GRID_DIRECT) && !defined(SDFK_ABLATE_BOUNDS)
+        float4 bb = meta->bound[sdfk_tx()];
+        if (meta->uniform[sdfk_tx()]) bb = sdfk_direct_centre<1>(meta, s.ax2, (int)g.L - 1, sdfk_tx(), 0u);
+#else
         const float4 bb = meta->bound[sdfk_tx()];
+#endif
         V3T<float> ctr = {bb.x, bb.y, bb.z};
         unsigned long long mk[SDFK_NMASK];
 #pragma unroll
@@ -1281,7 +1429,8 @@
 template <typename SRC>
 static __device__ __forceinline__ void sdfk_rows_kernel(const float* __restrict__ PRM, const float* __restrict__ TAB,
                                                         const SRC& s, const sdfk_rowgeom& g, float* __restrict__ out,
-                                                        unsigned* __restrict__ flags, unsigned thr SDFK_CELLS_PARAM) {
+                                                        unsigned* __restrict__ flags, unsigned thr SDFK_CELLS_PARAM
+                                                        SDFK_DIRECT_KARG) {
     __shared__ __attribute__((aligned(16))) sdfk_rowmeta meta;
 #ifdef SDFK_LDSPAD
     if (g.L == 0xffffffffu) meta.pad[sdfk_tx()] = 1.0f;
@@ -1309,7 +1458,10 @@
     if (tile * SDFK_RNBRICK >= g.nbricks) break;
     if (tt) __syncthreads();
     unsigned rb, c;
-    sdfk_rows_prepare(PRM, TAB, s, g, &meta, tile, rb, c SDFK_CELLS_PASS);
+#ifdef SDFK_GRID_DIRECT
+    sdfk_gridregs gr[SDFK_RWBRICKS];
+#endif
+    sdfk_rows_prepare(PRM, TAB, s, g, &meta, tile, rb, c SDFK_CELLS_PASS SDFK_DIRECT_PASS);
     const unsigned q0 = tile * SDFK_RNBRICK + wave * SDFK_RWBRICKS;
 #pragma unroll 1
     for (int j = 0; j < SDFK_RWBRICKS; ++j) {
@@ -1327,7 +1479,9 @@
             mw[2 * w] = __builtin_amdgcn_readfirstlane((unsigned)m);
             mw[2 * w + 1] = __builtin_amdgcn_readfirstlane((unsigned)(m >> 32));
         }
+#ifndef SDFK_GRID_DIRECT
         const bool uniform = __builtin_amdgcn_readfirstlane(meta.uniform[b]) != 0u;
+#endif
         const bool interior = sdfk_interior(g.L, k);
 #ifdef SDFK_ABLATE_EDGE
         if (!interior) continue;
@@ -1339,8 +1493,18 @@
         const int last = (int)g.L - 1;
         V3P P[SDFK_NP];
         f2 res[SDFK_NP];
+#ifdef SDFK_GRID_DIRECT
+        // the lane's own loads of brick j (j is wave-uniform: selects, the registers are never indexed)
+        float2 xy = gr[0].xy;
+        SDFK_EACH P[q].z = gr[0].z[q];
+#pragma unroll
+        for (int jj = 1; jj < SDFK_RWBRICKS; ++jj)
+            if (j == jj) {
+                xy = gr[jj].xy;
+                SDFK_EACH P[q].z = gr[jj].z[q];
+            }
+#elif defined(SDFK_FLAT)
         // the staged coordinate: z (SDFK_FLAT: y, see sdfk_rows_load)
-#ifdef SDFK_FLAT
         SDFK_EACH P[q].y = *reinterpret_cast<const f2*>(&meta.z[b][lr * SDFK_RZ + zq + 2 * q]);
 #else
         SDFK_EACH P[q].z = *reinterpret_cast<const f2*>(&meta.z[b][lr * SDFK_RZ + zq + 2 * q]);
@@ -1354,6 +1518,12 @@
 #endif
         } else
 #endif
+#ifdef SDFK_GRID_DIRECT
+        {
+            SDFK_EACH { P[q].x = sp<f2>(xy.x); P[q].y = sp<f2>(xy.y); }
+            sdfk_rows_culled<true>(xy.x, xy.y, P, mw, PRM, TAB, res);
+        }
+#else
         if (uniform) {
             const float2 xy = meta.xy[b][lr];
 #ifdef SDFK_FLAT
@@ -1383,6 +1553,7 @@
             sdfk_rows_culled<false>(0.0f, 0.0f, P, mw, PRM, TAB, res);
 #endif
         }
+#endif
 #ifdef SDFK_CHAIN
         {   // The children on the brick's list, in order; the first one starts the accumulator. Looked up one by one — kind of
             // the child, base of its parameters, then the parameters: three dependent scalar loads per child — the evaluation
@@ -1706,8 +1877,8 @@
 // starts at a row boundary and out[0] is its first point
 extern "C" __global__ __launch_bounds__(64 * SDFK_RWAVES) void sdfk_spec_rg(
     const float* __restrict__ PRM, const float* __restrict__ TAB, SrcGrid s, sdfk_rowgeom g, float* __restrict__ out,
-    unsigned* __restrict__ flags, unsigned thr SDFK_CELLS_KARG) {
-    sdfk_rows_kernel(PRM, TAB, s, g, out, flags, thr SDFK_CELLS_PASS);
+    unsigned* __restrict__ flags, unsigned thr SDFK_CELLS_KARG SDFK_DIRECT_KARG) {
+    sdfk_rows_kernel(PRM, TAB, s, g, out, flags, thr SDFK_CELLS_PASS SDFK_DIRECT_KPASS);
 }
 #ifdef SDFK_CELLS
 extern "C" __global__ __launch_bounds__(256) void sdfk_spec_cellsg(
@@ -2724,6 +2895,8 @@
         }
         g.emit_probe();
         g.emit_rows_culled(result_reg);
+        if (flavour == SDFK_FL_ROWS_GRID)
+            g.s += "#if !defined(SDFK_FLAGS) && !defined(SDFK_GRID_STAGED)\n#define SDFK_GRID_DIRECT 1\n#endif\n";
         g.s += kRowsKernel;
         if (all || flavour == SDFK_FL_ROWS_ARRAY || flavour == SDFK_FL_ROWS2D_ARRAY) g.s += kRowsArray;
         if (all || flavour == SDFK_FL_ROWS_GRID || flavour == SDFK_FL_ROWS2D_GRID) g.s += kRowsGrid;
diff --git a/aegolius_amd/csrc/sdfk_occupancy.inc b/aegolius_amd/csrc/sdfk_occupancy.inc
--- a/aegolius_amd/csrc/sdfk_occupancy.inc
+++ b/aegolius_amd/csrc/sdfk_occupancy.inc
@@ -253,7 +253,7 @@
         if (pass_ms) HIPCHK(hipEventRecord(ev.e[0], stream));
         if (skip) {
             g.start = first;
-            rc = run(p, nullptr, &g, cells, d_centre, stream, mode, true);
+            rc = run_grid(p, g, axes, cells, d_centre, stream, mode, true);
             if (rc) return rc;
             if (pass_ms) HIPCHK(hipEventRecord(ev.e[1], stream));
             C.first = first;
diff --git a/include/sdfk.h b/include/sdfk.h
--- a/include/sdfk.h
+++ b/include/sdfk.h
@@ -51,6 +51,7 @@
 void sdfk_jit_cancel(void);
 void sdfk_debug_jit_stats(int64_t* builds, double* seconds);
 void sdfk_debug_set_rtc_defs(const char* defs);
+int sdfk_debug_grid_rowsplit(int64_t row0, uint32_t n1, uint32_t r, uint64_t* ix, uint32_t* iy, uint32_t* inv_n1);
 
 int sdfk_eval_device(sdfk_program* prog, const float* d_co, int64_t n, int64_t row_stride, float* d_out,
                      void* stream, int mode);
```

After: 368,600. No clear change (-0.9%).
